# ming024/FastSpeech2

Hardware: AMD Instinct MI355X
Metric: mel-frames/sec (train, 80-bin) (higher is better)
Workload: dtype bf16; 1 GPU; BASELINE configs[1]: LJSpeech train, 4+4 FFT layers d=256 2 heads, 80-bin mel, batch=48/GPU, L=128 phonemes, T=925 frames, fwd+loss+bwd+clip+Adam, dropout on, fp32 master weights; global_batch=48, parallelism=dp1, hip_graph=False, side_stream_wgrad=True, windows=1, library=fastspeech2_amd/libfs2hip.so

## Files before the change

fastspeech2_amd/csrc/fs2_common.h:

```cpp
#pragma once
#include <hip/hip_runtime.h>
#include <stdint.h>
#include <stdio.h>
#include <mutex>
#include <stdlib.h>

#define FS2_OK 0
#define FS2_EINVAL (-1)
#define FS2_EDTYPE (-2)
#define FS2_ELAUNCH (-3)

enum { FS2_F32 = 0, FS2_BF16 = 1 };
enum { FS2_ACT_NONE = 0, FS2_ACT_RELU = 1, FS2_ACT_TANH = 2, FS2_ACT_LRELU = 3, FS2_ACT_GATE = 4 };

void fs2_set_error(const char* fmt, ...);

#define FS2_CHECK_ARG(cond, ...)                \
    do {                                        \
        if (!(cond)) {                          \
            fs2_set_error(__VA_ARGS__);         \
            return FS2_EINVAL;                  \
        }                                       \
    } while (0)

struct Fs2DevOnce {
    std::mutex mu;
    uint64_t done = 0;
    template <typename F>
    void run(F&& f) {
        int d = 0;
        (void)hipGetDevice(&d);
        const uint64_t bit = 1ull << (d & 63);
        std::lock_guard<std::mutex> g(mu);
        if (!(done & bit)) { f(); done |= bit; }
    }
};

#define FS2_CHECK_LAUNCH(name)                                                        \
    do {                                                                              \
        hipError_t e__ = hipGetLastError();                                           \
        if (e__ != hipSuccess) {                                                      \
            fs2_set_error("%s: launch failed: %s", name, hipGetErrorString(e__));     \
            return FS2_ELAUNCH;                                                       \
        }                                                                             \
    } while (0)

typedef uint16_t bf16_t;

__device__ __forceinline__ float bf16_to_f32(bf16_t v) { return __uint_as_float(((uint32_t)v) << 16); }
typedef __bf16 fs2_bf16x2 __attribute__((ext_vector_type(2)));
typedef float fs2_f32x2 __attribute__((ext_vector_type(2)));
__device__ __forceinline__ bf16_t f32_to_bf16(float f) { return __builtin_bit_cast(unsigned short, (__bf16)f); }
__device__ __forceinline__ uint32_t pack_bf16x2(float lo, float hi) {
    return __builtin_bit_cast(uint32_t, __builtin_convertvector((fs2_f32x2){lo, hi}, fs2_bf16x2));
}

template <typename T> struct Elem;
template <> struct Elem<float> {
    static __device__ __forceinline__ float ld(const float* p) { return *p; }
    static __device__ __forceinline__ void st(float* p, float v) { *p = v; }
};
template <> struct Elem<bf16_t> {
    static __device__ __forceinline__ float ld(const bf16_t* p) { return bf16_to_f32(*p); }
    static __device__ __forceinline__ void st(bf16_t* p, float v) { *p = f32_to_bf16(v); }
};

template <typename T> __device__ __forceinline__ float4 ld4(const T* p);
template <> __device__ __forceinline__ float4 ld4<float>(const float* p) { return *reinterpret_cast<const float4*>(p); }
template <> __device__ __forceinline__ float4 ld4<bf16_t>(const bf16_t* p) {
    uint2 u = *reinterpret_cast<const uint2*>(p);
    float4 r;
    r.x = __uint_as_float(u.x << 16);
    r.y = __uint_as_float(u.x & 0xffff0000u);
    r.z = __uint_as_float(u.y << 16);
    r.w = __uint_as_float(u.y & 0xffff0000u);
    return r;
}
template <typename T> __device__ __forceinline__ void st4(T* p, float4 v);
template <> __device__ __forceinline__ void st4<float>(float* p, float4 v) { *reinterpret_cast<float4*>(p) = v; }
template <> __device__ __forceinline__ void st4<bf16_t>(bf16_t* p, float4 v) {
    uint2 u;
    u.x = pack_bf16x2(v.x, v.y);
    u.y = pack_bf16x2(v.z, v.w);
    *reinterpret_cast<uint2*>(p) = u;
}

__device__ __forceinline__ float wave_sum(float v) {
#pragma unroll
    for (int o = 32; o > 0; o >>= 1) v += __shfl_xor(v, o, 64);
    return v;
}
__device__ __forceinline__ float wave_max(float v) {
#pragma unroll
    for (int o = 32; o > 0; o >>= 1) v = fmaxf(v, __shfl_xor(v, o, 64));
    return v;
}

__device__ __forceinline__ uint32_t fs2_hash32(uint32_t x) {
    x ^= x >> 16; x *= 0x7feb352du;
    x ^= x >> 15; x *= 0x846ca68bu;
    x ^= x >> 16;
    return x;
}
__device__ __forceinline__ float fs2_uniform(uint64_t seed, uint32_t idx) {
    uint32_t h = fs2_hash32(idx ^ (uint32_t)seed);
    h = fs2_hash32(h + (uint32_t)(seed >> 32) + 0x9e3779b9u);
    return (float)(h >> 8) * (1.0f / 16777216.0f);
}
__device__ __forceinline__ float fs2_drop_scale(uint64_t seed, uint32_t idx, float p, float inv_keep) {
    return (fs2_uniform(seed, idx) >= p) ? inv_keep : 0.0f;
}

#ifndef FS2_GEMM_PLAIN
#define FS2_GEMM_PLAIN 1
#define FS2_GEMM_DMA 2
#define FS2_GEMM_RING 3
#define FS2_GEMM_SKINNY 4
#define FS2_GEMM_PERSIST 5
#define FS2_GEMM_PERSIST_1TAP 6
#define FS2_GEMM_WIDE_1TAP 7
#define FS2_GEMM_STREAM_K256 9
#endif
static inline int fs2_cdiv(long a, long b) { return (int)((a + b - 1) / b); }
```

fastspeech2_amd/csrc/fs2_gemm.hip:

```cpp
#include "fs2_common.h"
#include <stdlib.h>
#include <type_traits>

#include "fs2_gemm.h"
#include "fs2_sched.h"
#include "fs2_wgrad.h"

template <typename T> __host__ __device__ __forceinline__ int fs2_tile_col128(int c) { return fs2_tile_col128_bytes((int)sizeof(T), c); }
template <typename T, int TW = 128, int NT = 256, int ROWS = 128>
__device__ __forceinline__ void gemm_store_tile(const ConvGemmArgs& a, const float* tile, int m0, int n0, int tid) {
    constexpr int EPC = MmaTraits<T>::EPC;
    T* Y = reinterpret_cast<T*>(a.Y);
    const T* R = reinterpret_cast<const T*>(a.R);
    constexpr int EPT = EPC;
    constexpr int CPR = TW / EPT;
    const bool gate = a.act == FS2_ACT_GATE;
#pragma unroll 4
    for (int it = 0; it < (ROWS * CPR) / NT; ++it) {
        int idx = tid + NT * it;
        int rl = idx / CPR, cc = (idx % CPR) * EPT;
        int m = m0 + rl, n = n0 + cc;
        if (m >= a.M || n >= a.N) continue;
        float v[EPT];
#pragma unroll
// ... 497 lines not shown

template <bool ONE_TAP, bool MASK, bool INACT>
__device__ __forceinline__ void ring_consumer(const ConvGemmArgs& a, unsigned char* smem, f32x16 (&acc)[2][2], int m0, int lane,
                                              int wm, int wn) {
    typedef RingCfg<ONE_TAP> C;
    constexpr int D = C::D;
    const int nkc = a.Cin >> 6;
    const int taps = ONE_TAP ? 1 : a.taps;
    const int nsteps = taps * nkc;
    const int fl = lane & 31, fh = lane >> 5;
    unsigned boff[4];
#pragma unroll
    for (int j = 0; j < 4; ++j) {
        int r = wn * 64 + fl;
        boff[j] = r * 128 + (((fh * 4 + j) ^ ((r >> 1) & 7)) << 4);
    }
    unsigned vmask[2] = {0, 0};
    if (MASK) {
#pragma unroll
        for (int mb = 0; mb < 2; ++mb) {
            int m = m0 + wm * 64 + mb * 32 + fl;
            unsigned msk = 0;
            if (m < a.M) {
                int t = m % a.S;
                for (int j = 0; j < taps; ++j) {
                    int ts = t + j * a.dil - a.pad;
                    if (ts >= 0 && ts < a.S) msk |= 1u << j;
                }
            }
            vmask[mb] = msk;
        }
    }
    typedef unsigned u32x4 __attribute__((ext_vector_type(4)));
#define FS2_DS_READ_B128(dst, addr, OFF) asm volatile("ds_read_b128 %0, %1 offset:" #OFF : "=v"(dst) : "v"(addr))
    u32x4 af[2][2][2], bf[2][2][2];
    const unsigned smem_u = lds_addr(smem);
    auto read_group = [&](int set, int kc, int tap, int slot, int g) {
        const int roff = tap * a.dil;
        const unsigned a_base = (ONE_TAP ? slot : (kc & 1)) * C::A_BYTES + (wm * 64 + roff) * 128;
        const unsigned x = ((fl + roff) >> 1) & 7;
#pragma unroll
        for (int q = 0; q < 2; ++q) {
            const int j = 2 * g + q;
            const unsigned aaddr = smem_u + a_base + fl * 128 + ((((unsigned)(fh * 4 + j)) ^ x) << 4);
            const unsigned baddr = smem_u + C::B_OFF + slot * RING_B_BYTES + boff[j];
            FS2_DS_READ_B128(bf[set][q][0], baddr, 0);
            FS2_DS_READ_B128(bf[set][q][1], baddr, 4096);
            FS2_DS_READ_B128(af[set][q][0], aaddr, 0);
            FS2_DS_READ_B128(af[set][q][1], aaddr, 4096);
        }
    };
    auto mfma_group = [&](int set, int tap) {
#pragma unroll
        for (int q = 0; q < 2; ++q)
#pragma unroll
            for (int mb = 0; mb < 2; ++mb) {
                u32x4 av = af[set][q][mb];
                if (INACT) {
#pragma unroll
                    for (int e = 0; e < 4; ++e) {
                        float lo = __uint_as_float(av[e] << 16), hi = __uint_as_float(av[e] & 0xffff0000u);
                        av[e] = pack_bf16x2(fmaxf(lo, lo * a.in_slope), fmaxf(hi, hi * a.in_slope));
                    }
                }
                if (MASK && !((vmask[mb] >> tap) & 1u)) av = u32x4{0u, 0u, 0u, 0u};
#pragma unroll
                for (int nb = 0; nb < 2; ++nb)
                    acc[mb][nb] = __builtin_amdgcn_mfma_f32_32x32x16_bf16(
                        __builtin_bit_cast(bf16x8, av), __builtin_bit_cast(bf16x8, bf[set][q][nb]), acc[mb][nb], 0, 0, 0);
            }
    };
    asm volatile("s_waitcnt lgkmcnt(0)" ::: "memory");
    __builtin_amdgcn_s_barrier();
    read_group(0, 0, 0, 0, 0);
    int slot = 0, step = 0;
    for (int kc = 0; kc < nkc; ++kc) {
        for (int tap = 0; tap < taps; ++tap, ++step) {
            read_group(1, kc, tap, slot, 1);
            asm volatile("s_waitcnt lgkmcnt(8)" ::: "memory");
            __builtin_amdgcn_sched_barrier(0);
            mfma_group(0, tap);
            __builtin_amdgcn_sched_barrier(0);
            int nslot = slot + 1; if (nslot == D) nslot = 0;
            int ntap = tap + 1, nkc_ = kc; if (ntap == taps) { ntap = 0; ++nkc_; }
            asm volatile("s_waitcnt lgkmcnt(0)" ::: "memory");
            if (step + 1 < nsteps) {
                __builtin_amdgcn_s_barrier();
                read_group(0, nkc_, ntap, nslot, 0);
            }
            __builtin_amdgcn_sched_barrier(0);
            mfma_group(1, tap);
            __builtin_amdgcn_sched_barrier(0);
            slot = nslot;
        }
    }
#undef FS2_DS_READ_B128
}

template <bool ONE_TAP, bool INACT>
__global__ void __launch_bounds__(768, 3) conv_gemm_ring_kernel(ConvGemmArgs a) {
    extern __shared__ __attribute__((aligned(16))) unsigned char smem[];
    const int tid = threadIdx.x, lane = tid & 63;
    const int wave = __builtin_amdgcn_readfirstlane(tid >> 6);
    const int wm = (wave >> 1) & 3, wn = wave & 1;
    const int ntm = (a.M + 255) >> 8;
    const int tile_m = blockIdx.x % ntm, tile_n = blockIdx.x / ntm;
    const int m0 = tile_m * 256, n0 = tile_n * 128;
    bf16_t* Y = reinterpret_cast<bf16_t*>(a.Y);

    if (a.lens) {
        int mlast = min(m0 + 255, a.M - 1);
        int b0 = m0 / a.S, b1 = mlast / a.S;
        if (b0 == b1 && (m0 - b0 * a.S) >= a.lens[b0]) {
            if (!a.accumulate) {
                for (int i = tid; i < 256 * 16; i += 768) {
                    int r = i >> 4, c = (i & 15) * 8;
                    int m = m0 + r, n = n0 + c;
                    if (m >= a.M || n >= a.N) continue;
                    bf16_t* yp = Y + (size_t)m * a.ldy + n;
                    if (a.vec_ok && n + 8 <= a.N) *reinterpret_cast<uint4*>(yp) = make_uint4(0, 0, 0, 0);
                    else for (int e = 0; e < 8 && n + e < a.N; ++e) yp[e] = 0;
                }
            }
            return;
        }
    }
    f32x16 acc[2][2];
    if (wave >= 8) {
        ring_loader<ONE_TAP>(a, smem, m0, n0, lane, wave - 8);
    } else {
#pragma unroll
        for (int i = 0; i < 2; ++i)
#pragma unroll
            for (int j = 0; j < 2; ++j)
#pragma unroll
                for (int r = 0; r < 16; ++r) acc[i][j][r] = 0.f;
        if (ONE_TAP) {
            ring_consumer<true, false, INACT>(a, smem, acc, m0, lane, wm, wn);
        } else {
            int t0 = m0 % a.S;
            int rows = min(256, a.M - m0);
            const bool need_mask = (t0 < a.pad) || (t0 + rows - 1 + (a.taps - 1) * a.dil - a.pad >= a.S);
            if (need_mask) ring_consumer<false, true, INACT>(a, smem, acc, m0, lane, wm, wn);
            else ring_consumer<false, false, INACT>(a, smem, acc, m0, lane, wm, wn);
        }
    }
    __syncthreads();

    float* tile = reinterpret_cast<float*>(smem);
    if (wave < 8) {
        const int fl = lane & 31, fh = lane >> 5;
        auto stage = [&](auto actc) {
            constexpr int ACT = decltype(actc)::value;
#pragma unroll
            for (int nb = 0; nb < 2; ++nb) {
                int cl = wn * 64 + nb * 32 + fl;
                int n = n0 + cl;
                float bv = (a.bias && n < a.N) ? a.bias[n] : 0.f;
#pragma unroll
                for (int mb = 0; mb < 2; ++mb)
#pragma unroll
                    for (int r = 0; r < 16; ++r) {
                        int rl = wm * 64 + mb * 32 + (r & 3) + 8 * (r >> 2) + 4 * fh;
                        tile[rl * 128 + fs2_tile_col128<bf16_t>(cl)] = act_ct<ACT>(acc[mb][nb][r] + bv, a.slope);
                    }
            }
        };
        FS2_ACT_DISPATCH(a.act, stage(std::integral_constant<int, ACT>{}));
    }
    __syncthreads();
    if (tid < 512) {
        gemm_store_tile<bf16_t, 128, 512>(a, tile, m0, n0, tid);
        gemm_store_tile<bf16_t, 128, 512>(a, tile + 128 * 128, m0 + 128, n0, tid);
    }
}

template <int C> struct SkinnyCfg {
    static constexpr int CPR = C / 8, RPW = 16 / CPR, XR_MAX = 192;
    static constexpr int G = C == 32 ? 8 : 2;
    static constexpr int X_BYTES = XR_MAX * C * 2, W_BYTES = G * C * C * 2;
    static constexpr int EPI_BYTES = 128 * C * 4;
    static constexpr int LDS = (X_BYTES + W_BYTES) > EPI_BYTES ? (X_BYTES + W_BYTES) : EPI_BYTES;
};
template <int C> __device__ __forceinline__ unsigned skinny_swz(int row, int c) {
    typedef SkinnyCfg<C> K;
    return (unsigned)(row * (C * 2) + ((c ^ ((row / K::RPW) % K::CPR)) << 4));
}

template <int C>
__global__ void __launch_bounds__(256) conv_skinny_kernel(ConvGemmArgs a) {
    typedef SkinnyCfg<C> K;
    constexpr int CPR = K::CPR, NB = C / 32, NS = C / 16;
    extern __shared__ __attribute__((aligned(16))) unsigned char smem[];
    unsigned char* sX = smem;
    unsigned char* sW = smem + K::X_BYTES;
    const int tid = threadIdx.x, lane = tid & 63, fl = lane & 31, fh = lane >> 5;
    const int wave = __builtin_amdgcn_readfirstlane(tid >> 6);
    const int m0 = blockIdx.x * 128;
    const bf16_t* X = reinterpret_cast<const bf16_t*>(a.X);
    const bf16_t* W = reinterpret_cast<const bf16_t*>(a.W);
    const int halo = (a.taps - 1) * a.dil;
    const int xr = 128 + halo;
    constexpr int MAXI = (K::XR_MAX * CPR + 255) / 256;
    uint4 xv[MAXI];
#pragma unroll
    for (int i = 0; i < MAXI; ++i) {
        const int idx = tid + 256 * i;
        const int row = idx / CPR, c = idx % CPR;
        const int g = m0 - a.pad + row;
        uint4 v = make_uint4(0, 0, 0, 0);
        if (row < xr && g >= 0 && g < a.M) v = *reinterpret_cast<const uint4*>(X + (size_t)g * a.ldx + c * 8);
        xv[i] = v;
    }
#pragma unroll
    for (int i = 0; i < MAXI; ++i) {
        const int idx = tid + 256 * i;
        const int row = idx / CPR, c = idx % CPR;
        if (row < xr) {
            uint4 v = xv[i];
            if (a.in_act == FS2_ACT_LRELU) v = act_chunk_bf16(v, a.in_slope);
            *reinterpret_cast<uint4*>(sX + skinny_swz<C>(row, c)) = v;
        }
    }
    unsigned vmask = 0;
    {
        const int m = m0 + wave * 32 + fl;
        if (m < a.M) {
            const int t = m % a.S;
            for (int j = 0; j < a.taps; ++j) {
                const int ts = t + j * a.dil - a.pad;
                if (ts >= 0 && ts < a.S) vmask |= 1u << j;
            }
        }
    }
    f32x16 acc[NB];
#pragma unroll
    for (int nb = 0; nb < NB; ++nb)
#pragma unroll
        for (int r = 0; r < 16; ++r) acc[nb][r] = 0.f;

    constexpr int WI = (K::G * C * CPR) / 256;
    for (int g0 = 0; g0 < a.taps; g0 += K::G) {
        __syncthreads();
#pragma unroll
        for (int i = 0; i < WI; ++i) {
            const int idx = tid + 256 * i;
            const int tl = idx / (C * CPR), rem = idx % (C * CPR);
            const int n = rem / CPR, c = rem % CPR;
            uint4 v = make_uint4(0, 0, 0, 0);
            if (g0 + tl < a.taps) v = *reinterpret_cast<const uint4*>(W + ((size_t)n * a.taps + (g0 + tl)) * C + c * 8);
            *reinterpret_cast<uint4*>(sW + tl * (C * C * 2) + skinny_swz<C>(n, c)) = v;
        }
        __syncthreads();
#pragma unroll
        for (int tl = 0; tl < K::G; ++tl) {
            const int tap = g0 + tl;
            if (tap >= a.taps) break;
            const int r = wave * 32 + fl + tap * a.dil;
            const bool live = (vmask >> tap) & 1u;
            const unsigned char* wt = sW + tl * (C * C * 2);
#pragma unroll
            for (int sl = 0; sl < NS; ++sl) {
                const int c = 2 * sl + fh;
                uint4 av = *reinterpret_cast<const uint4*>(sX + skinny_swz<C>(r, c));
                if (!live) av = make_uint4(0, 0, 0, 0);
#pragma unroll
                for (int nb = 0; nb < NB; ++nb) {
                    uint4 bv = *reinterpret_cast<const uint4*>(wt + skinny_swz<C>(nb * 32 + fl, c));
                    acc[nb] = __builtin_amdgcn_mfma_f32_32x32x16_bf16(__builtin_bit_cast(bf16x8, av), __builtin_bit_cast(bf16x8, bv), acc[nb], 0, 0, 0);
                }
            }
        }
    }
    __syncthreads();
    float* tile = reinterpret_cast<float*>(smem);
    auto stage = [&](auto actc) {
        constexpr int ACT = decltype(actc)::value;
#pragma unroll
        for (int nb = 0; nb < NB; ++nb) {
            const int cl = nb * 32 + fl;
            const float bv = a.bias ? a.bias[cl] : 0.f;
#pragma unroll
            for (int r = 0; r < 16; ++r) {
                const int rl = wave * 32 + (r & 3) + 8 * (r >> 2) + 4 * fh;
                tile[rl * C + cl] = act_ct<ACT>(acc[nb][r] + bv, a.slope);
            }
        }
    };
    FS2_ACT_DISPATCH(a.act, stage(std::integral_constant<int, ACT>{}));
    __syncthreads();
    gemm_store_tile<bf16_t, C, 256, 128>(a, tile, m0, 0, tid);
}

template <int C>
static void launch_skinny(const ConvGemmArgs& a, hipStream_t stream) {
    static Fs2DevOnce once;
    once.run([&] { (void)hipFuncSetAttribute((const void*)conv_skinny_kernel<C>, hipFuncAttributeMaxDynamicSharedMemorySize, SkinnyCfg<C>::LDS); });
    conv_skinny_kernel<C><<<(unsigned)fs2_cdiv(a.M, 128), 256, SkinnyCfg<C>::LDS, stream>>>(a);
}

bool fs2_conv_gemm_w_ok(const ConvGemmArgs& a, bool has_map, int dtype);
void fs2_conv_gemm_w_launch(const ConvGemmArgs& a, const int32_t* tile_map, hipStream_t stream);
bool fs2_conv_gemm_p_ok(const ConvGemmArgs& a, bool has_map, int dtype, int ks);
void fs2_conv_gemm_p_launch(const ConvGemmArgs& a, const int32_t* tile_map, hipStream_t stream, int ks, float* ws, float* tail_ws);

bool fs2_conv_gemm_s_ok(const ConvGemmArgs& a, int dtype);
void fs2_conv_gemm_s_launch(const ConvGemmArgs& a, hipStream_t stream);
struct GemmPick { int variant; bool ring_inact, ks2; };
static GemmPick conv_gemm_pick(const ConvGemmArgs& a, int dtype, bool has_map, bool has_tail_ws = true) {
    const int M = a.M, N = a.N, Cin = a.Cin, taps = a.taps, dil = a.dil, in_act = a.in_act;
    GemmPick p;
    const long grid = (long)fs2_cdiv(M, 128) * fs2_cdiv(N, 128);
    const bool dma = in_act == FS2_ACT_NONE && (taps > 1 || (grid <= 160 && Cin % 128 == 0 && Cin >= 768 && dtype == FS2_BF16)) && (taps - 1) * dil <= 16 && taps <= 32;
    const long big_tiles = (long)fs2_cdiv(M, 256) * fs2_cdiv(N, 128);
    p.ring_inact = in_act == FS2_ACT_LRELU && a.in_slope > 0.f && a.in_slope < 1.f;
    const bool ring_ok = dtype == FS2_BF16 && (in_act == FS2_ACT_NONE || p.ring_inact) && (taps == 1 || (taps >= 3 && (taps - 1) * dil <= 16 && taps <= 32)) &&
                         Cin % 64 == 0 && (double)M * a.ldx * 2 < 2.0e9 && (double)N * taps * Cin * 2 < 2.0e9;
    const bool big = ring_ok && big_tiles >= 170 && (taps > 1 || Cin >= 1024);
    const bool skinny = dtype == FS2_BF16 && N == Cin && (Cin == 32 || Cin == 64) && taps <= 16 &&
                        (taps - 1) * dil <= 64 && (in_act == FS2_ACT_NONE || in_act == FS2_ACT_LRELU) && a.vec_ok;
    const bool res_short = (a.res_unlrelu > 0.f || a.post_slope > 0.f) && (a.R || a.accumulate) && a.act != FS2_ACT_GATE &&
                           (long)taps * ((Cin + 63) / 64) <= 48 && big;
    const bool persist = !skinny && !res_short && fs2_conv_gemm_p_ok(a, has_map, dtype, 1) && (taps > 1 || Cin >= 256);
    p.ks2 = dtype == FS2_BF16 && grid <= 160 && Cin % 128 == 0 && (long)taps * (Cin / 64) >= 12;
    const bool lrelu_io = a.res_unlrelu > 0.f || a.post_slope > 0.f;
    if (!skinny && !lrelu_io && fs2_conv_gemm_s_ok(a, dtype)) { p.variant = FS2_GEMM_STREAM_K256; return p; }
    if (!skinny && fs2_conv_gemm_w_ok(a, has_map, dtype)) { p.variant = FS2_GEMM_WIDE_1TAP; return p; }
    p.variant = skinny ? FS2_GEMM_SKINNY : (persist ? (taps == 1 ? FS2_GEMM_PERSIST_1TAP : FS2_GEMM_PERSIST) : (big ? FS2_GEMM_RING : (dma ? FS2_GEMM_DMA : FS2_GEMM_PLAIN)));
    return p;
}

static void conv_gemm_fill(ConvGemmArgs& a, const void* X, long ldx, const void* W, const float* bias, const void* R, long ldr, void* Y,
                           long ldy, const int32_t* lens, int M, int N, int Cin, int S, int taps, int dil, int pad, int act, float slope,
                           int in_act, float in_slope, int accumulate, float out_scale, int dtype) {
    const int epc = dtype == FS2_F32 ? 4 : 8;
    a.X = X; a.ldx = ldx; a.W = W; a.ldw = (long)taps * Cin; a.bias = bias; a.R = R; a.ldr = ldr; a.Y = Y; a.ldy = ldy;
    a.lens = lens; a.M = M; a.N = N; a.Cin = Cin; a.S = S; a.taps = taps; a.dil = dil; a.pad = pad; a.act = act;
    a.slope = slope; a.in_act = in_act; a.in_slope = in_slope; a.accumulate = accumulate; a.out_scale = out_scale;
    a.res_unlrelu = 0.f; a.post_slope = 0.f;
    a.vec_ok = (ldy % epc == 0) && (((uintptr_t)Y & 15) == 0) && (!R || ((ldr % epc == 0) && (((uintptr_t)R & 15) == 0)));
}

extern "C" int fs2_conv_gemm_variant(long ldx, long ldy, long ldr, int has_lens, int has_map, int M, int N, int Cin, int S, int taps,
                                     int dil, int in_act, float in_slope, int dtype) {
    ConvGemmArgs a;
    conv_gemm_fill(a, nullptr, ldx, nullptr, nullptr, ldr ? (const void*)16 : nullptr, ldr, nullptr, ldy, has_lens ? (const int32_t*)16 : nullptr,
                   M, N, Cin, S > 0 ? S : 1, taps, dil, 0, 0, 0.f, in_act, in_slope, 0, 1.f, dtype);
    return conv_gemm_pick(a, dtype, has_map != 0).variant;
}

extern "C" int fs2_conv_gemm_lrelu_io_variant(long ldx, long ldy, long ldr, int accumulate, int M, int N, int Cin, int S, int taps, int dil,
                                              int act, float res_unlrelu, float post_slope, int dtype) {
    ConvGemmArgs a;
    conv_gemm_fill(a, nullptr, ldx, nullptr, nullptr, ldr ? (const void*)16 : nullptr, ldr, nullptr, ldy, nullptr, M, N, Cin, S > 0 ? S : 1,
                   taps, dil, 0, act, 0.f, FS2_ACT_NONE, 0.f, accumulate, 1.f, dtype);
    a.res_unlrelu = res_unlrelu; a.post_slope = post_slope;
    return conv_gemm_pick(a, dtype, false).variant;
}

static int conv_gemm_impl(const void* X, long ldx, const void* W, const float* bias, const void* R, long ldr, void* Y,
                          long ldy, const int32_t* lens, const int32_t* tile_map, float* tail_ws, int M, int N, int Cin, int S, int taps,
                          int dil, int pad, int act, float slope, int in_act, float in_slope, int accumulate, float out_scale,
                          int dtype, hipStream_t stream, float res_unlrelu = 0.f, float post_slope = 0.f) {
    FS2_CHECK_ARG(X && W && Y, "conv_gemm: null pointer");
    FS2_CHECK_ARG(M >= 0 && N > 0 && Cin > 0 && S > 0 && taps > 0 && dil > 0, "conv_gemm: bad shape M=%d N=%d Cin=%d S=%d taps=%d", M, N, Cin, S, taps);
    FS2_CHECK_ARG(M % S == 0, "conv_gemm: M=%d not a multiple of S=%d", M, S);
    int epc = dtype == FS2_F32 ? 4 : 8;
    FS2_CHECK_ARG(dtype == FS2_F32 || dtype == FS2_BF16, "conv_gemm: dtype %d", dtype);
    FS2_CHECK_ARG(Cin % epc == 0 && ldx % epc == 0, "conv_gemm: Cin=%d / ldx=%ld must be multiples of %d", Cin, ldx, epc);
    FS2_CHECK_ARG(((uintptr_t)X & 15) == 0 && ((uintptr_t)W & 15) == 0, "conv_gemm: X/W must be 16-byte aligned");
    if (M == 0) return FS2_OK;
    ConvGemmArgs a;
    conv_gemm_fill(a, X, ldx, W, bias, R, ldr, Y, ldy, lens, M, N, Cin, S, taps, dil, pad, act, slope, in_act, in_slope, accumulate, out_scale, dtype);
    FS2_CHECK_ARG(res_unlrelu >= 0.f && post_slope >= 0.f && post_slope < 1.f && (res_unlrelu == 0.f || (R && act != FS2_ACT_GATE)),
                  "conv_gemm: res_unlrelu needs an additive residual operand, post_slope in [0, 1)");
    a.res_unlrelu = res_unlrelu; a.post_slope = post_slope;
    const long grid = (long)fs2_cdiv(M, 128) * fs2_cdiv(N, 128);
    const long big_tiles = (long)fs2_cdiv(M, 256) * fs2_cdiv(N, 128);
    const GemmPick pk = conv_gemm_pick(a, dtype, tile_map != nullptr, tail_ws != nullptr);
    if (pk.variant == FS2_GEMM_STREAM_K256) {
        fs2_conv_gemm_s_launch(a, stream);
    } else if (pk.variant == FS2_GEMM_SKINNY) {
        if (Cin == 32) launch_skinny<32>(a, stream);
        else launch_skinny<64>(a, stream);
    } else if (pk.variant == FS2_GEMM_WIDE_1TAP) {
        fs2_conv_gemm_w_launch(a, tile_map, stream);
    } else if (pk.variant == FS2_GEMM_PERSIST || pk.variant == FS2_GEMM_PERSIST_1TAP) {
        fs2_conv_gemm_p_launch(a, tile_map, stream, 1, nullptr, tail_ws);
    } else if (pk.variant == FS2_GEMM_RING) {
        static Fs2DevOnce ring_once;
        const int dyn1 = RingCfg<true>::B_OFF + RingCfg<true>::D * RING_B_BYTES;
        const int dynk = RingCfg<false>::B_OFF + RingCfg<false>::D * RING_B_BYTES;
        ring_once.run([&] {
            (void)hipFuncSetAttribute((const void*)conv_gemm_ring_kernel<true, false>, hipFuncAttributeMaxDynamicSharedMemorySize, dyn1);
            (void)hipFuncSetAttribute((const void*)conv_gemm_ring_kernel<false, false>, hipFuncAttributeMaxDynamicSharedMemorySize, dynk);
            (void)hipFuncSetAttribute((const void*)conv_gemm_ring_kernel<true, true>, hipFuncAttributeMaxDynamicSharedMemorySize, dyn1);
            (void)hipFuncSetAttribute((const void*)conv_gemm_ring_kernel<false, true>, hipFuncAttributeMaxDynamicSharedMemorySize, dynk);
        });
        if (pk.ring_inact) {
            if (taps == 1) conv_gemm_ring_kernel<true, true><<<(unsigned)big_tiles, 768, dyn1, stream>>>(a);
            else conv_gemm_ring_kernel<false, true><<<(unsigned)big_tiles, 768, dynk, stream>>>(a);
        } else if (taps == 1) conv_gemm_ring_kernel<true, false><<<(unsigned)big_tiles, 768, dyn1, stream>>>(a);
        else conv_gemm_ring_kernel<false, false><<<(unsigned)big_tiles, 768, dynk, stream>>>(a);
    } else if (pk.variant == FS2_GEMM_DMA) {
        const int dyn = 2 * 160 * 128 + 2 * 128 * 128;
        static Fs2DevOnce dma_once;
        dma_once.run([&] {
            (void)hipFuncSetAttribute((const void*)conv_gemm_dma_kernel<float, 1>, hipFuncAttributeMaxDynamicSharedMemorySize, dyn);
            (void)hipFuncSetAttribute((const void*)conv_gemm_dma_kernel<bf16_t, 1>, hipFuncAttributeMaxDynamicSharedMemorySize, dyn);
            (void)hipFuncSetAttribute((const void*)conv_gemm_dma_kernel<bf16_t, 2>, hipFuncAttributeMaxDynamicSharedMemorySize, 2 * dyn);
        });
        if (dtype == FS2_F32) conv_gemm_dma_kernel<float, 1><<<(unsigned)grid, 256, dyn, stream>>>(a);
        else if (pk.ks2) conv_gemm_dma_kernel<bf16_t, 2><<<(unsigned)grid, 512, 2 * dyn, stream>>>(a);
        else conv_gemm_dma_kernel<bf16_t, 1><<<(unsigned)grid, 256, dyn, stream>>>(a);
    } else if (dtype == FS2_F32) conv_gemm_kernel<float><<<(unsigned)grid, 256, 0, stream>>>(a);
    else conv_gemm_kernel<bf16_t><<<(unsigned)grid, 256, 0, stream>>>(a);
    FS2_CHECK_LAUNCH("conv_gemm");
    return FS2_OK;
}

extern "C" int fs2_conv_gemm(const void* X, long ldx, const void* W, const float* bias, const void* R, long ldr, void* Y,
                             long ldy, const int32_t* lens, const int32_t* tile_map, int M, int N, int Cin, int S, int taps, int dil,
                             int pad, int act, float slope, int in_act, float in_slope, int accumulate, float out_scale, int dtype,
                             hipStream_t stream) {
    return conv_gemm_impl(X, ldx, W, bias, R, ldr, Y, ldy, lens, tile_map, nullptr, M, N, Cin, S, taps, dil, pad, act, slope, in_act,
                          in_slope, accumulate, out_scale, dtype, stream);
}

extern "C" int fs2_conv_gemm_tail(const void* X, long ldx, const void* W, const float* bias, const void* R, long ldr, void* Y,
                                  long ldy, const int32_t* lens, const int32_t* tile_map, float* tail_ws, int M, int N, int Cin,
                                  int S, int taps, int dil, int pad, int act, float slope, int in_act, float in_slope,
                                  int accumulate, float out_scale, int dtype, hipStream_t stream) {
    FS2_CHECK_ARG(!tail_ws || ((uintptr_t)tail_ws & 15) == 0, "conv_gemm_tail: tail_ws must be 16-byte aligned");
    return conv_gemm_impl(X, ldx, W, bias, R, ldr, Y, ldy, lens, tile_map, tail_ws, M, N, Cin, S, taps, dil, pad, act, slope, in_act,
                          in_slope, accumulate, out_scale, dtype, stream);
}

extern "C" int fs2_conv_gemm_lrelu_io(const void* X, long ldx, const void* W, const float* bias, const void* R, long ldr, void* Y,
                                      long ldy, float* tail_ws, int M, int N, int Cin, int S, int taps, int dil, int pad, int act,
                                      float slope, int accumulate, float out_scale, float res_unlrelu, float post_slope, int dtype,
                                      hipStream_t stream) {
    FS2_CHECK_ARG(!tail_ws || ((uintptr_t)tail_ws & 15) == 0, "conv_gemm_lrelu_io: tail_ws must be 16-byte aligned");
    return conv_gemm_impl(X, ldx, W, bias, R, ldr, Y, ldy, nullptr, nullptr, tail_ws, M, N, Cin, S, taps, dil, pad, act, slope,
                          FS2_ACT_NONE, 0.f, accumulate, out_scale, dtype, stream, res_unlrelu, post_slope);
}

extern "C" int fs2_conv_gemm_splitk(const void* X, long ldx, const void* W, const float* bias, const void* R, long ldr, void* Y,
                                    long ldy, const int32_t* lens, const int32_t* tile_map, float* ws, int ksplit, int M, int N,
                                    int Cin, int S, int taps, int dil, int pad, int act, float slope, float out_scale, int dtype,
                                    hipStream_t stream) {
    FS2_CHECK_ARG(X && W && Y && ws, "conv_gemm_splitk: null pointer");
    FS2_CHECK_ARG(M > 0 && N > 0 && Cin > 0 && S > 0 && taps > 0 && dil > 0 && M % S == 0 && ksplit >= 2, "conv_gemm_splitk: bad shape");
    FS2_CHECK_ARG(((uintptr_t)X & 15) == 0 && ((uintptr_t)W & 15) == 0 && ((uintptr_t)ws & 15) == 0 && ldx % 8 == 0, "conv_gemm_splitk: alignment");
    ConvGemmArgs a;
    conv_gemm_fill(a, X, ldx, W, bias, R, ldr, Y, ldy, lens, M, N, Cin, S, taps, dil, pad, act, slope, FS2_ACT_NONE, 0.f, 0, out_scale, dtype);
    FS2_CHECK_ARG(fs2_conv_gemm_p_ok(a, tile_map != nullptr, dtype, ksplit), "conv_gemm_splitk: shape not supported (M=%d N=%d Cin=%d taps=%d ksplit=%d)", M, N, Cin, taps, ksplit);
    fs2_conv_gemm_p_launch(a, tile_map, stream, ksplit, ws, nullptr);
    FS2_CHECK_LAUNCH("conv_gemm_splitk");
    return FS2_OK;
}

template <typename T>
__global__ void pack_weight_kernel(const float* __restrict__ w, T* __restrict__ wf, T* __restrict__ wd, int Cout, int Cin, int k) {
    size_t total = (size_t)Cout * Cin * k;
    for (size_t i = (size_t)blockIdx.x * blockDim.x + threadIdx.x; i < total; i += (size_t)gridDim.x * blockDim.x) {
        int c = (int)(i % Cin);
        size_t q = i / Cin;
        int j = (int)(q % k);
        int n = (int)(q / k);
        float v = w[i];
        if (wf) Elem<T>::st(wf + i, v);
        if (wd) Elem<T>::st(wd + ((size_t)c * k + (k - 1 - j)) * Cout + n, v);
    }
}
extern "C" int fs2_pack_weight(const float* w, void* wf, void* wd, int Cout, int Cin, int k, int dtype, hipStream_t stream) {
    FS2_CHECK_ARG(w && (wf || wd), "pack_weight: null pointer");
    size_t total = (size_t)Cout * Cin * k;
    if (total == 0) return FS2_OK;
    int grid = (int)((total + 255) / 256 < 4096 ? (total + 255) / 256 : 4096);
    if (dtype == FS2_F32) pack_weight_kernel<float><<<grid, 256, 0, stream>>>(w, (float*)wf, (float*)wd, Cout, Cin, k);
    else if (dtype == FS2_BF16) pack_weight_kernel<bf16_t><<<grid, 256, 0, stream>>>(w, (bf16_t*)wf, (bf16_t*)wd, Cout, Cin, k);
    else { fs2_set_error("pack_weight: dtype"); return FS2_EDTYPE; }
    FS2_CHECK_LAUNCH("pack_weight");
    return FS2_OK;
}

template <typename T>
__global__ void __launch_bounds__(256) pack_dgrad_multi_kernel(const float* __restrict__ flat, T* __restrict__ wd_base,
                                                               const int64_t* __restrict__ table, int n_entries) {
    __shared__ float tile[64][65];
    int e = 0;
    while (e + 1 < n_entries && (int)table[(e + 1) * 6 + 5] <= (int)blockIdx.x) ++e;
    const int64_t* d = table + e * 6;
    const float* w = flat + d[0];
    T* wd = wd_base + d[1];
    const int Cout = (int)d[2], Cin = (int)d[3], k = (int)d[4];
    int t = (int)blockIdx.x - (int)d[5];
    const int tn = (Cout + 63) >> 6, tc = (Cin + 63) >> 6;
    const int in_ = t % tn; t /= tn;
    const int ic = t % tc; t /= tc;
    const int j = t;
    const int n0 = in_ * 64, c0 = ic * 64;
    const int lx = threadIdx.x & 63, ly = threadIdx.x >> 6;
#pragma unroll 4
    for (int r = ly; r < 64; r += 4) {
        int n = n0 + r, c = c0 + lx;
        tile[r][lx] = (n < Cout && c < Cin) ? w[((size_t)n * k + j) * Cin + c] : 0.f;
    }
    __syncthreads();
#pragma unroll 4
    for (int r = ly; r < 64; r += 4) {
        int c = c0 + r, n = n0 + lx;
        if (c < Cin && n < Cout) Elem<T>::st(wd + ((size_t)c * k + (k - 1 - j)) * Cout + n, tile[lx][r]);
    }
}
extern "C" int fs2_pack_dgrad_multi(const float* flat, void* wd_base, const int64_t* table, int n_entries, int total_tiles,
                                    int dtype, hipStream_t stream) {
    FS2_CHECK_ARG(flat && wd_base && table, "pack_dgrad_multi: null pointer");
    if (n_entries <= 0 || total_tiles <= 0) return FS2_OK;
    if (dtype == FS2_F32) pack_dgrad_multi_kernel<float><<<total_tiles, 256, 0, stream>>>(flat, (float*)wd_base, table, n_entries);
    else if (dtype == FS2_BF16) pack_dgrad_multi_kernel<bf16_t><<<total_tiles, 256, 0, stream>>>(flat, (bf16_t*)wd_base, table, n_entries);
    else { fs2_set_error("pack_dgrad_multi: dtype"); return FS2_EDTYPE; }
    FS2_CHECK_LAUNCH("pack_dgrad_multi");
    return FS2_OK;
}


template <typename T>
__global__ void __launch_bounds__(256, 2) conv_wgrad_kernel(WgradArgs a) {
    __shared__ __attribute__((aligned(16))) float sA[2][32][128];
    __shared__ __attribute__((aligned(16))) float sB[2][32][128];
    const int tid = threadIdx.x, lane = tid & 63, wave = tid >> 6;
    const int wm = wave >> 1, wn = wave & 1;
    const int ntn = (a.N + 127) >> 7, ntc = (a.Cin + 127) >> 7;
    int bx = blockIdx.x;
    const int tile_n = bx % ntn; bx /= ntn;
    const int tile_c = bx % ntc; bx /= ntc;
    const int tap = bx;
    const int n0 = tile_n * 128, c0 = tile_c * 128;
    const int shift = tap * a.dil - a.pad;
    const int mbeg = blockIdx.y * a.rows_per_split;
    const int mend = min(a.M, mbeg + a.rows_per_split);
    if (mbeg >= mend) return;
    const T* dY = reinterpret_cast<const T*>(a.dY);
    const T* X = reinterpret_cast<const T*>(a.X);

    const int sr = tid >> 5, sc4 = (tid & 31) * 4;
    float4 ra[4], rb[4];
    auto load_tile = [&](int mt) {
#pragma unroll
        for (int i = 0; i < 4; ++i) {
            int m = mt + sr + 8 * i;
            float4 va = make_float4(0.f, 0.f, 0.f, 0.f), vb = va;
            if (m < mend) {
                int n = n0 + sc4;
                if (n < a.N) va = ld4<T>(dY + (size_t)m * a.lddy + n);
                int t = m % a.S, ts = t + shift;
                int c = c0 + sc4;
                if (ts >= 0 && ts < a.S && c < a.Cin) vb = ld4<T>(X + (size_t)(m + shift) * a.ldx + c);
            }
            ra[i] = va; rb[i] = vb;
        }
    };
    auto store_tile = [&](int buf) {
#pragma unroll
        for (int i = 0; i < 4; ++i) {
            *reinterpret_cast<float4*>(&sA[buf][sr + 8 * i][sc4]) = ra[i];
            *reinterpret_cast<float4*>(&sB[buf][sr + 8 * i][sc4]) = rb[i];
        }
    };
    f32x16 acc[2][2];
#pragma unroll
    for (int i = 0; i < 2; ++i)
#pragma unroll
        for (int j = 0; j < 2; ++j)
#pragma unroll
            for (int r = 0; r < 16; ++r) acc[i][j][r] = 0.f;
    const int fl = lane & 31, fh = lane >> 5;
    int nt = (mend - mbeg + 31) / 32;
    load_tile(mbeg);
    store_tile(0);
    __syncthreads();
    for (int it = 0; it < nt; ++it) {
        if (it + 1 < nt) load_tile(mbeg + (it + 1) * 32);
        int buf = it & 1;
#pragma unroll
        for (int ks = 0; ks < 16; ++ks) {
            float af[2], bf[2];
            int row = ks * 2 + fh;
#pragma unroll
            for (int mb = 0; mb < 2; ++mb) af[mb] = sA[buf][row][wm * 64 + mb * 32 + fl];
#pragma unroll
            for (int nb = 0; nb < 2; ++nb) bf[nb] = sB[buf][row][wn * 64 + nb * 32 + fl];
#pragma unroll
            for (int mb = 0; mb < 2; ++mb)
#pragma unroll
                for (int nb = 0; nb < 2; ++nb)
                    acc[mb][nb] = __builtin_amdgcn_mfma_f32_32x32x2f32(af[mb], bf[nb], acc[mb][nb], 0, 0, 0);
        }
        if (it + 1 < nt) store_tile((it + 1) & 1);
        __syncthreads();
    }
#pragma unroll
    for (int nb = 0; nb < 2; ++nb) {
        int c = c0 + wn * 64 + nb * 32 + fl;
        if (c >= a.Cin) continue;
#pragma unroll
        for (int mb = 0; mb < 2; ++mb)
#pragma unroll
            for (int r = 0; r < 16; ++r) {
                int n = n0 + wm * 64 + mb * 32 + (r & 3) + 8 * (r >> 2) + 4 * fh;
                if (n >= a.N) continue;
                atomicAdd(a.dW + ((size_t)n * a.taps + tap) * a.Cin + c, acc[mb][nb][r]);
            }
    }
}


typedef short s16x4 __attribute__((ext_vector_type(4)));
typedef short s16x8 __attribute__((ext_vector_type(8)));

__device__ __forceinline__ uint4 and4(uint4 v, unsigned m) { return make_uint4(v.x & m, v.y & m, v.z & m, v.w & m); }
__device__ __forceinline__ int wg_swz(int row, int c16) { return row * 256 + ((((c16 >> 2) ^ (row & 3))) << 6) + ((c16 & 3) << 4); }

template <int NT, int NW>
__device__ __forceinline__ void wgrad_bf16_body(const WgradArgs& a, unsigned char* smem, int tile_n, int tile_c, int tap0) {
    constexpr int XROWS = 64 + 8;
    constexpr int A_BYTES = 64 * 256, X_BYTES = XROWS * 256;
    const int tid = threadIdx.x, lane = tid & 63;
    const int wave = __builtin_amdgcn_readfirstlane(tid >> 6);
    constexpr int NBC = NW == 4 ? 2 : 1;
    constexpr int RS = NW * 4, NI = 64 / RS;
    const int wm = NW == 4 ? (wave >> 1) : (wave >> 2), wn = NW == 4 ? (wave & 1) : (wave & 3);
    const int n0 = tile_n * 128, c0 = tile_c * 128;
    const int shift0 = tap0 * a.dil - a.pad;
    const int tps = (a.S + 63) >> 6;
    const int nunits = (a.M / a.S) * tps;
    const int ubeg = blockIdx.y * a.rows_per_split;
    const int uend = min(nunits, ubeg + a.rows_per_split);
    if (ubeg >= uend) return;
    const bf16_t* dY = reinterpret_cast<const bf16_t*>(a.dY);
    const bf16_t* X = reinterpret_cast<const bf16_t*>(a.X);

    const int sr = tid >> 4, sc = tid & 15;
    const bool ncol_ok = (n0 + sc * 8) < a.N, ccol_ok = (c0 + sc * 8) < a.Cin;
    const int ncol = ncol_ok ? n0 + sc * 8 : 0, ccol = ccol_ok ? c0 + sc * 8 : 0;
    const bool x5 = wave < 2;
    uint4 ra[2][NI], rb[2][NI], rb4[2] = {make_uint4(0, 0, 0, 0), make_uint4(0, 0, 0, 0)};
    bool live_t[2] = {false, false};
    const bool do_bias = a.dbias != nullptr && tile_c == 0 && tap0 == 0;
    float bsum[8] = {0.f, 0.f, 0.f, 0.f, 0.f, 0.f, 0.f, 0.f};
    const bool col_full = (n0 + 128 <= a.N) && (c0 + 128 <= a.Cin);
    const unsigned char* dYb = reinterpret_cast<const unsigned char*>(dY);
    const unsigned char* Xb = reinterpret_cast<const unsigned char*>(X);
    const unsigned dy_rs = (unsigned)a.lddy * 2u, x_rs = (unsigned)a.ldx * 2u;
    unsigned okmask_t[2] = {0, 0};
    bool edge_t[2] = {false, false};
    auto load_tile = [&](auto setc, int u) {
        constexpr int SET = decltype(setc)::value;
        const bool valid = u < uend;
        const int uu = valid ? u : ubeg;
        const int seq = uu / tps, t0 = (uu - seq * tps) * 64;
        const int tend = a.lens ? min(a.lens[seq], a.S) : a.S;
        live_t[SET] = valid && t0 < tend;
        edge_t[SET] = !col_full || (t0 + 64 > tend) || (t0 + shift0 < 0) || (t0 + shift0 + XROWS > a.S);
        const unsigned base = (unsigned)(seq * a.S);
        unsigned ok = 0;
#pragma unroll
        for (int i = 0; i < NI; ++i) {
            const int t = t0 + sr + RS * i;
            const size_t o = (size_t)(base + (unsigned)min(t, a.S - 1)) * dy_rs + (unsigned)ncol * 2u;
            ra[SET][i] = *reinterpret_cast<const uint4*>(dYb + o);
            ok |= (ncol_ok && t < tend) ? (1u << i) : 0u;
        }
#pragma unroll
        for (int i = 0; i < NI; ++i) {
            const int t = t0 + shift0 + sr + RS * i;
            const size_t o = (size_t)(base + (unsigned)min(max(t, 0), a.S - 1)) * x_rs + (unsigned)ccol * 2u;
            rb[SET][i] = *reinterpret_cast<const uint4*>(Xb + o);
            ok |= (ccol_ok && t >= 0 && t < a.S) ? (16u << i) : 0u;
        }
        {
            const int t = t0 + shift0 + sr + 64;
            const size_t o = (size_t)(base + (unsigned)min(max(t, 0), a.S - 1)) * x_rs + (unsigned)ccol * 2u;
            rb4[SET] = *reinterpret_cast<const uint4*>(Xb + o);
            ok |= (ccol_ok && t >= 0 && t < a.S) ? 256u : 0u;
        }
        okmask_t[SET] = ok;
    };
    auto store_tile = [&](auto setc, int buf) {
        constexpr int SET = decltype(setc)::value;
        const unsigned okmask = okmask_t[SET];
        unsigned char* As = smem + buf * (A_BYTES + X_BYTES);
        unsigned char* Bs = As + A_BYTES;
        if (edge_t[SET]) {
#pragma unroll
            for (int i = 0; i < NI; ++i) ra[SET][i] = and4(ra[SET][i], 0u - ((okmask >> i) & 1u));
#pragma unroll
            for (int i = 0; i < NI; ++i) rb[SET][i] = and4(rb[SET][i], 0u - ((okmask >> (4 + i)) & 1u));
            rb4[SET] = and4(rb4[SET], 0u - ((okmask >> 8) & 1u));
        }
#pragma unroll
        for (int i = 0; i < NI; ++i) *reinterpret_cast<uint4*>(As + wg_swz(sr + RS * i, sc)) = ra[SET][i];
#pragma unroll
        for (int i = 0; i < NI; ++i) *reinterpret_cast<uint4*>(Bs + wg_swz(sr + RS * i, sc)) = rb[SET][i];
        if (x5) *reinterpret_cast<uint4*>(Bs + wg_swz(sr + 64, sc)) = rb4[SET];
        if (do_bias) {
#pragma unroll
            for (int i = 0; i < NI; ++i) {
                const uint32_t* u32 = reinterpret_cast<const uint32_t*>(&ra[SET][i]);
#pragma unroll
                for (int e = 0; e < 4; ++e) {
                    bsum[2 * e] += __uint_as_float(u32[e] << 16);
                    bsum[2 * e + 1] += __uint_as_float(u32[e] & 0xffff0000u);
                }
            }
        }
    };
    f32x16 acc[NT][2][NBC];
#pragma unroll
    for (int t = 0; t < NT; ++t)
#pragma unroll
        for (int i = 0; i < 2; ++i)
#pragma unroll
            for (int j = 0; j < NBC; ++j)
#pragma unroll
                for (int r = 0; r < 16; ++r) acc[t][i][j][r] = 0.f;
    const int li = lane & 15, g = lane >> 4, h = g >> 1;
    const int rrow = 8 * h + (li >> 2);
    const int acol = wm * 64 + 16 * (g & 1) + 4 * (li & 3);
    const int bcol = wn * (32 * NBC) + 16 * (g & 1) + 4 * (li & 3);
    typedef __attribute__((address_space(3))) s16x4* lds_s4;
    auto tr_off = [&](int row, int col) -> unsigned { return (unsigned)(row * 256 + ((((col >> 5) ^ (row & 3))) << 6) + ((col & 31) << 1)); };
    unsigned offA[2][2], offB[NT][NBC][2];
#pragma unroll
    for (int blk = 0; blk < 2; ++blk)
#pragma unroll
        for (int hl = 0; hl < 2; ++hl) {
            offA[blk][hl] = tr_off(rrow + 4 * hl, acol + blk * 32);
            if (blk < NBC) {
#pragma unroll
                for (int t = 0; t < NT; ++t) offB[t][blk][hl] = A_BYTES + tr_off(rrow + 4 * hl + t * a.dil, bcol + blk * 32);
            }
        }
    const unsigned smem_u = (unsigned)(size_t)(__attribute__((address_space(3))) unsigned char*)smem;
    auto tr_read = [&](unsigned off) -> s16x4 {
        return __builtin_amdgcn_ds_read_tr16_b64_v4i16((lds_s4)(size_t)(smem_u + off));
    };
    s16x8 af[2][2], bf[2][NT][NBC];
    auto read_frags = [&](int set, int bufoff, int ks) {
#pragma unroll
        for (int blk = 0; blk < 2; ++blk) {
            s16x4 lo = tr_read(offA[blk][0] + bufoff + ks * 4096);
            s16x4 hi = tr_read(offA[blk][1] + bufoff + ks * 4096);
            af[set][blk] = __builtin_shufflevector(lo, hi, 0, 1, 2, 3, 4, 5, 6, 7);
        }
#pragma unroll
        for (int t = 0; t < NT; ++t)
#pragma unroll
            for (int blk = 0; blk < NBC; ++blk) {
                s16x4 lo = tr_read(offB[t][blk][0] + bufoff + ks * 4096);
// ... 268 lines not shown
```

fastspeech2_amd/csrc/fs2_gemm_p.hip:

```cpp
#include "fs2_gemm.h"
#include "fs2_sched.h"
#include "fs2_gemm_epi.h"


template <bool ONE_TAP, bool WIDE> struct PCfg;
template <> struct PCfg<false, false> {
    static constexpr int D = 5, HALO = 16, A_BYTES = 272 * 128, SCRATCH = 2 * 272 * 128, B_OFF = 2 * 272 * 128 + 1024, NJA = 9;
    static constexpr int AUX = B_OFF + D * 16384;
};
template <> struct PCfg<false, true> {
    static constexpr int D = 4, HALO = 64, A_BYTES = 320 * 128, SCRATCH = 2 * 320 * 128, B_OFF = 2 * 320 * 128 + 1024, NJA = 10;
    static constexpr int AUX = B_OFF + D * 16384;
};
template <> struct PCfg<true, false> {
    static constexpr int D = 3, HALO = 0, A_BYTES = 256 * 128, SCRATCH = 0, B_OFF = 3 * 256 * 128, NJA = 8;
    static constexpr int AUX = B_OFF + D * 16384;
};
__device__ __forceinline__ const unsigned char* p_uniform(const unsigned char* q) {
    const unsigned long long u = reinterpret_cast<unsigned long long>(q);
    const unsigned lo = __builtin_amdgcn_readfirstlane((unsigned)u), hi = __builtin_amdgcn_readfirstlane((unsigned)(u >> 32));
    return reinterpret_cast<const unsigned char*>(((unsigned long long)hi << 32) | lo);
}
template <int N> __device__ __forceinline__ void p_wait_vm() { asm volatile("s_waitcnt vmcnt(%0)" :: "n"(N) : "memory"); }
static constexpr int P_MAXB = 1024;
static constexpr int P_AUX_BYTES = P_MAXB * 4 + 8 * 512;
static constexpr int P_B_BYTES = 128 * 128;

__device__ __forceinline__ int p_ntiles(const PSched& s) {
    const PPlan p = p_plan(s, s.b);
    return p.R + (p.j < p.tail * p.tks ? 1 : 0);
}
__device__ __forceinline__ int p_last_nkc(const PSched& s) {
    const PPlan p = p_plan(s, s.b);
    return (p.j < p.tail * p.tks) ? s.nkc_u / p.tks : s.nkc_u;
}

struct PUnits { unsigned v0, v1; };
__device__ __forceinline__ void p_units_load(const PSched& s, int lane, PUnits& t) {
    int mi, nt, kc0, nkc, np;
    unsigned a0 = 0, a1 = 0;
    if (p_unit(s, lane, mi, nt, kc0, nkc, np)) {
        const int mt = s.tmap ? s.tmap[1 + mi] : mi;
        a0 = (unsigned)mt | ((unsigned)nt << 20) | ((unsigned)np << 28);
        a1 = (unsigned)kc0 | ((unsigned)nkc << 16);
    }
    t.v0 = a0; t.v1 = a1;
}
__device__ __forceinline__ void p_tile_of(const PSched& s, int k, const PUnits& t, int& mt, int& nt, int& kc0, int* split = nullptr,
                                          int* nparts = nullptr) {
    const unsigned a0 = __builtin_amdgcn_readlane(t.v0, k), a1 = __builtin_amdgcn_readlane(t.v1, k);
    mt = (int)(a0 & 0xfffffu);
    nt = (int)((a0 >> 20) & 0xffu);
    kc0 = __builtin_amdgcn_readfirstlane((int)(a1 & 0xffffu));
    if (nparts) *nparts = (int)(a0 >> 28);
    if (split) *split = kc0 / s.nkc_u;
}

template <bool ONE_TAP, bool WIDE>
__device__ __forceinline__ void p_loader(const ConvGemmArgs& a, const PSched& sc, unsigned char* smem, int lane, int lw,
                                         const PUnits& units, int ntiles) {
    typedef PCfg<ONE_TAP, WIDE> C;
    constexpr int D = C::D, NJA = C::NJA;
    const unsigned char* Xb = reinterpret_cast<const unsigned char*>(a.X);
    const unsigned char* Wb = reinterpret_cast<const unsigned char*>(a.W);
    const int nkc = sc.nkc_u;
    const int nkc_last = p_last_nkc(sc);
    const int taps = ONE_TAP ? 1 : a.taps;
    const int nsteps = taps * nkc;
    const int total = (ntiles - 1) * nsteps + taps * nkc_last;
    const int nchunks = (ntiles - 1) * nkc + nkc_last;
    int kc0A = 0, kc0B = 0;
    const int lr = lane >> 3, lc = lane & 7;
    const int arows = 256 + (taps - 1) * a.dil;
    const unsigned smem_base = lds_addr(smem);

    unsigned offA[NJA], ldsA[NJA], offB[4];
    auto set_A = [&](int k) {
        int mt, nt;
        p_tile_of(sc, k, units, mt, nt, kc0A);
        const int m0 = mt * 256;
#pragma unroll
        for (int j = 0; j < NJA; ++j) {
            const int wl = lw + 4 * j;
            const bool live = wl * 8 < arows;
            const int r = wl * 8 + lr;
            const int g = min(max(m0 - a.pad + r, 0), a.M - 1);
            offA[j] = live ? (unsigned)g * (unsigned)(a.ldx * 2) + (unsigned)((lc ^ ((r >> 1) & 7)) << 4) : 0u;
            ldsA[j] = live ? (unsigned)(wl * 1024) : 0xffffffffu;
        }
    };
    auto set_B = [&](int k) {
        int mt, nt;
        p_tile_of(sc, k, units, mt, nt, kc0B);
        const int n0 = nt * 128;
#pragma unroll
        for (int j = 0; j < 4; ++j) {
            const int r = (lw * 4 + j) * 8 + lr;
            const int n = min(n0 + r, a.N - 1);
            offB[j] = (unsigned)n * (unsigned)(a.ldw * 2) + (unsigned)((lc ^ ((r >> 1) & 7)) << 4);
        }
    };
    int is = 0, ik = 0, ikc = 0, itap = 0, islot = 0;
    int kA = -1, kB = -1;
    auto issue_A = [&](int k, int kc, int buf_or_slot) {
        if (k != kA) { set_A(k); kA = k; }
        const unsigned char* base = p_uniform(Xb + (size_t)(kc0A + kc) * 128);
#pragma unroll
        for (int j = 0; j < NJA; ++j) {
            const unsigned d = (ldsA[j] == 0xffffffffu) ? smem_base + C::SCRATCH : smem_base + buf_or_slot * C::A_BYTES + ldsA[j];
            glds16_sbase(offA[j], base, __builtin_amdgcn_readfirstlane(d));
        }
    };
    auto issue_step = [&]() {
        if (ik != kB) { set_B(ik); kB = ik; }
        if (ONE_TAP) issue_A(ik, ikc, islot);
        const unsigned char* base = p_uniform(Wb + ((size_t)itap * a.Cin + (size_t)(kc0B + ikc) * 64) * 2);
        const unsigned d0 = smem_base + C::B_OFF + islot * P_B_BYTES + lw * 4096;
#pragma unroll
        for (int j = 0; j < 4; ++j) glds16_sbase(offB[j], base, d0 + j * 1024);
    };
    auto advance_issue = [&]() {
        ++is;
        if (++itap == taps) { itap = 0; if (++ikc == (ik == ntiles - 1 ? nkc_last : nkc)) { ikc = 0; ++ik; } }
        if (++islot == D) islot = 0;
    };
    if (!ONE_TAP) issue_A(0, 0, 0);
#pragma unroll
    for (int p = 0; p < D - 1; ++p) {
        if (is < total) issue_step();
        advance_issue();
    }
    int ck = 0, ckc = 0, ctap = 0, gc = 0;
    for (int cs = 0; cs < total; ++cs) {
        if (total - 1 - cs < D - 2) {
            asm volatile("s_waitcnt vmcnt(0)" ::: "memory");
        } else if (ONE_TAP) {
            p_wait_vm<(D - 2) * (NJA + 4)>();
        } else {
            const bool a_young = (ctap >= 1 && ctap <= D - 2) && (gc + 1 < nchunks);
            if (a_young) p_wait_vm<(D - 2) * 4 + NJA>();
            else p_wait_vm<(D - 2) * 4>();
        }
        __builtin_amdgcn_s_barrier();
        if (!ONE_TAP && ctap == 0 && gc + 1 < nchunks) {
            int nk = ck, nkc_ = ckc + 1;
            if (nkc_ == (ck == ntiles - 1 ? nkc_last : nkc)) { nkc_ = 0; ++nk; }
            issue_A(nk, nkc_, (gc + 1) & 1);
        }
        if (is < total) issue_step();
        advance_issue();
        if (++ctap == taps) { ctap = 0; ++gc; if (++ckc == (ck == ntiles - 1 ? nkc_last : nkc)) { ckc = 0; ++ck; } }
    }
}

#define FS2P_DS_READ(dst, addr, OFF) asm volatile("ds_read_b128 %0, %1 offset:" #OFF : "=v"(dst) : "v"(addr))
#define FS2P_WAIT_LGKM(N) asm volatile("s_waitcnt lgkmcnt(" #N ")" ::: "memory")
#define FS2P_FENCE() __builtin_amdgcn_sched_barrier(0)

template <int MB>
__device__ __forceinline__ void p_epilogue_splitk(const ConvGemmArgs& a, float* ws, f32x16 (&acc)[MB][4], int m0, int n0, int wm,
                                                  int fl, int fh) {
#pragma unroll
    for (int mb = 0; mb < MB; ++mb) {
        const int m = m0 + wm * (32 * MB) + mb * 32 + fl;
        if (m >= a.M) continue;
        float* wrow = ws + (size_t)m * a.N;
#pragma unroll
        for (int nb = 0; nb < 4; ++nb) {
            float c[2][8];
#pragma unroll
            for (int e = 0; e < 4; ++e) {
                u32x2 s0 = __builtin_amdgcn_permlane32_swap(__float_as_uint(acc[mb][nb][e]), __float_as_uint(acc[mb][nb][4 + e]), false, false);
                u32x2 s1 = __builtin_amdgcn_permlane32_swap(__float_as_uint(acc[mb][nb][8 + e]), __float_as_uint(acc[mb][nb][12 + e]), false, false);
                c[0][e] = __uint_as_float(s0[0]); c[0][4 + e] = __uint_as_float(s0[1]);
                c[1][e] = __uint_as_float(s1[0]); c[1][4 + e] = __uint_as_float(s1[1]);
            }
#pragma unroll
            for (int ch = 0; ch < 2; ++ch) {
                const int n = n0 + nb * 32 + ch * 16 + fh * 8;
                if (n >= a.N) continue;
                *reinterpret_cast<float4*>(wrow + n) = make_float4(c[ch][0], c[ch][1], c[ch][2], c[ch][3]);
                *reinterpret_cast<float4*>(wrow + n + 4) = make_float4(c[ch][4], c[ch][5], c[ch][6], c[ch][7]);
            }
        }
    }
}

template <int ACT>
__global__ void __launch_bounds__(256) splitk_finalize_kernel(ConvGemmArgs a, const float* __restrict__ ws, int ks) {
    const int cpr = a.N >> 3;
    const long idx = (long)blockIdx.x * 256 + threadIdx.x;
    if (idx >= (long)a.M * cpr) return;
    const int m = (int)(idx / cpr), n = (int)(idx - (long)m * cpr) * 8;
    const float* wp = ws + (size_t)m * a.N + n;
    const size_t slab = (size_t)a.M * a.N;
    float v[8] = {0.f, 0.f, 0.f, 0.f, 0.f, 0.f, 0.f, 0.f};
    for (int sp = 0; sp < ks; ++sp) {
        const float4 x0 = *reinterpret_cast<const float4*>(wp + sp * slab), x1 = *reinterpret_cast<const float4*>(wp + sp * slab + 4);
        v[0] += x0.x; v[1] += x0.y; v[2] += x0.z; v[3] += x0.w; v[4] += x1.x; v[5] += x1.y; v[6] += x1.z; v[7] += x1.w;
    }
    if (a.bias) {
#pragma unroll
        for (int e = 0; e < 8; ++e) v[e] += a.bias[n + e];
    }
#pragma unroll
    for (int e = 0; e < 8; ++e) v[e] = act_ct<ACT>(v[e], a.slope);
    const bool gate = a.act == FS2_ACT_GATE;
    if (a.R) {
        const uint4 rv = *reinterpret_cast<const uint4*>(reinterpret_cast<const bf16_t*>(a.R) + (size_t)m * a.ldr + n);
        const uint32_t* u = reinterpret_cast<const uint32_t*>(&rv);
#pragma unroll
        for (int e = 0; e < 4; ++e) {
            float r0 = __uint_as_float(u[e] << 16), r1 = __uint_as_float(u[e] & 0xffff0000u);
            if (a.res_unlrelu > 0.f) { r0 = r0 > 0.f ? r0 : r0 * a.res_unlrelu; r1 = r1 > 0.f ? r1 : r1 * a.res_unlrelu; }
            v[2 * e] = gate ? (r0 > 0.f ? v[2 * e] : 0.f) : v[2 * e] + r0;
            v[2 * e + 1] = gate ? (r1 > 0.f ? v[2 * e + 1] : 0.f) : v[2 * e + 1] + r1;
        }
    }
    bool padrow = false;
    if (a.lens) { const int b = m / a.S; padrow = (m - b * a.S) >= a.lens[b]; }
    uint4 o;
    uint32_t* ou = reinterpret_cast<uint32_t*>(&o);
#pragma unroll
    for (int e = 0; e < 4; ++e) {
        float x0 = v[2 * e] * a.out_scale, x1 = v[2 * e + 1] * a.out_scale;
        if (a.post_slope > 0.f) { x0 = x0 > 0.f ? x0 : x0 * a.post_slope; x1 = x1 > 0.f ? x1 : x1 * a.post_slope; }
        ou[e] = padrow ? 0u : pack_bf16x2(x0, x1);
    }
    *reinterpret_cast<uint4*>(reinterpret_cast<bf16_t*>(a.Y) + (size_t)m * a.ldy + n) = o;
}

template <int MB>
__device__ __forceinline__ void p_epilogue_part(float* slab, f32x16 (&acc)[MB][4], int wm, int fl, int fh) {
#pragma unroll
    for (int mb = 0; mb < MB; ++mb) {
        float* wrow = slab + (size_t)(wm * (32 * MB) + mb * 32 + fl) * 128;
#pragma unroll
        for (int nb = 0; nb < 4; ++nb) {
            float c[2][8];
#pragma unroll
            for (int e = 0; e < 4; ++e) {
                u32x2 s0 = __builtin_amdgcn_permlane32_swap(__float_as_uint(acc[mb][nb][e]), __float_as_uint(acc[mb][nb][4 + e]), false, false);
                u32x2 s1 = __builtin_amdgcn_permlane32_swap(__float_as_uint(acc[mb][nb][8 + e]), __float_as_uint(acc[mb][nb][12 + e]), false, false);
                c[0][e] = __uint_as_float(s0[0]); c[0][4 + e] = __uint_as_float(s0[1]);
                c[1][e] = __uint_as_float(s1[0]); c[1][4 + e] = __uint_as_float(s1[1]);
            }
#pragma unroll
            for (int ch = 0; ch < 2; ++ch) {
                const int n = nb * 32 + ch * 16 + fh * 8;
                *reinterpret_cast<float4*>(wrow + n) = make_float4(c[ch][0], c[ch][1], c[ch][2], c[ch][3]);
                *reinterpret_cast<float4*>(wrow + n + 4) = make_float4(c[ch][4], c[ch][5], c[ch][6], c[ch][7]);
            }
        }
    }
}

template <int ACT>
__global__ void __launch_bounds__(256) p_tail_finalize_kernel(ConvGemmArgs a, PSched sc) {
    const int i = blockIdx.y;
    sc.b = sc.order == 0 ? 2 * i : (i & 7) + 8 * (2 * (i >> 3));
    if (sc.b >= sc.G) return;
    if (sc.tmap) { sc.n_real = sc.tmap[0]; sc.n_pad = sc.ntm - sc.n_real; }
    const PPlan p = p_plan(sc, sc.b);
    if (p.tks <= 1 || p.j >= p.tail * p.tks || (p.j % p.tks) != 0) return;
    int mi, nt, sp;
    p_pos(sc, p, p.R * p.Gg + p.j / p.tks, mi, nt, sp);
    const int mt = sc.tmap ? sc.tmap[1 + mi] : mi;
    const bool gate = a.act == FS2_ACT_GATE;
#pragma unroll
  for (int pass = 0; pass < 4; ++pass) {
    const int idx = (blockIdx.x * 4 + pass) * 256 + threadIdx.x;
    const int r = idx >> 4, cn = (idx & 15) * 8;
    const int m = mt * 256 + r, n = nt * 128 + cn;
    if (m >= a.M || n >= a.N) continue;
    float v[8] = {0.f, 0.f, 0.f, 0.f, 0.f, 0.f, 0.f, 0.f};
    for (int q = 0; q < p.tks; ++q) {
        const int wg = sc.order == 0 ? sc.b + q : p.x + 8 * (p.j + q);
        const float* sl = sc.tws + (size_t)wg * (256 * 128) + r * 128 + cn;
        const float4 x0 = *reinterpret_cast<const float4*>(sl), x1 = *reinterpret_cast<const float4*>(sl + 4);
        v[0] += x0.x; v[1] += x0.y; v[2] += x0.z; v[3] += x0.w; v[4] += x1.x; v[5] += x1.y; v[6] += x1.z; v[7] += x1.w;
    }
    if (a.bias) {
#pragma unroll
        for (int e = 0; e < 8; ++e) v[e] += a.bias[n + e];
    }
#pragma unroll
    for (int e = 0; e < 8; ++e) v[e] = act_ct<ACT>(v[e], a.slope);
    if (a.R) {
        const uint4 rv = *reinterpret_cast<const uint4*>(reinterpret_cast<const bf16_t*>(a.R) + (size_t)m * a.ldr + n);
        const uint32_t* u = reinterpret_cast<const uint32_t*>(&rv);
#pragma unroll
        for (int e = 0; e < 4; ++e) {
            float r0 = __uint_as_float(u[e] << 16), r1 = __uint_as_float(u[e] & 0xffff0000u);
            if (a.res_unlrelu > 0.f) { r0 = r0 > 0.f ? r0 : r0 * a.res_unlrelu; r1 = r1 > 0.f ? r1 : r1 * a.res_unlrelu; }
            v[2 * e] = gate ? (r0 > 0.f ? v[2 * e] : 0.f) : v[2 * e] + r0;
            v[2 * e + 1] = gate ? (r1 > 0.f ? v[2 * e + 1] : 0.f) : v[2 * e + 1] + r1;
        }
    }
    bool padrow = false;
    if (a.lens) { const int b = m / a.S; padrow = (m - b * a.S) >= a.lens[b]; }
    uint4 o;
    uint32_t* ou = reinterpret_cast<uint32_t*>(&o);
#pragma unroll
    for (int e = 0; e < 4; ++e) {
        float x0 = v[2 * e] * a.out_scale, x1 = v[2 * e + 1] * a.out_scale;
        if (a.post_slope > 0.f) { x0 = x0 > 0.f ? x0 : x0 * a.post_slope; x1 = x1 > 0.f ? x1 : x1 * a.post_slope; }
        ou[e] = padrow ? 0u : pack_bf16x2(x0, x1);
    }
    *reinterpret_cast<uint4*>(reinterpret_cast<bf16_t*>(a.Y) + (size_t)m * a.ldy + n) = o;
  }
}

__device__ __forceinline__ u32x4 p_lrelu(u32x4 v, float slope) {
#pragma unroll
    for (int e = 0; e < 4; ++e) {
        const float lo = __uint_as_float(v[e] << 16), hi = __uint_as_float(v[e] & 0xffff0000u);
        v[e] = pack_bf16x2(fmaxf(lo, lo * slope), fmaxf(hi, hi * slope));
    }
    return v;
}

template <bool ONE_TAP, bool WIDE, int INACT, int MB>
__device__ __forceinline__ void p_consumer(const ConvGemmArgs& a, const PSched& sc, unsigned char* smem, int lane, int wm,
                                           const PUnits& units, int ntiles, const int32_t* lens_s, float* bias_s) {
    typedef PCfg<ONE_TAP, WIDE> C;
    constexpr int D = C::D;
    const int nkc = sc.nkc_u;
    const int nkc_last = p_last_nkc(sc);
    const int taps = ONE_TAP ? 1 : a.taps;
    const int nsteps = taps * nkc;
    const int total = (ntiles - 1) * nsteps + taps * nkc_last;
    const int fl = lane & 31, fh = lane >> 5;
    const unsigned smem_u = lds_addr(smem);
    const unsigned c0 = (unsigned)(fh * 4);
    const unsigned ckb = c0 ^ (unsigned)((fl >> 1) & 7);
    const unsigned blane = smem_u + C::B_OFF + (unsigned)(fl * 128);
    const unsigned alane = smem_u + (unsigned)((wm * (32 * MB) + fl) * 128);
    auto a_base = [&](int abuf, int tap) -> unsigned { return alane + (unsigned)(abuf * C::A_BYTES + tap * a.dil * 128); };
    auto a_key = [&](int tap) -> unsigned { return c0 ^ (unsigned)(((fl + tap * a.dil) >> 1) & 7); };
    auto b_base = [&](int slot) -> unsigned { return blane + (unsigned)(slot * P_B_BYTES); };

    u32x4 Af[2][MB], Bf[2][4];
    f32x16 acc[MB][4];

#define FS2P_MFMA(SET, MB, NB, AV)                                                                                      \
    acc[MB][NB] = __builtin_amdgcn_mfma_f32_32x32x16_bf16(__builtin_bit_cast(bf16x8, Bf[SET][NB]), __builtin_bit_cast(bf16x8, AV), \
                                                          acc[MB][NB], 0, 0, 0)
#define FS2P_SLICE(SET, MASKED, LIVE0, LIVE1, JN, ABASE, AKEY, BBASE)                                                   \
    do {                                                                                                                \
        u32x4 av0, av1;                                                                                                 \
        FS2P_WAIT_LGKM(4); FS2P_FENCE();                                                                                \
        av0 = Af[SET][0]; if (INACT) av0 = p_lrelu(av0, a.in_slope);                                                    \
        if (MASKED && !(LIVE0)) av0 = u32x4{0u, 0u, 0u, 0u};                                                            \
        FS2P_MFMA(SET, 0, 0, av0); FS2P_FENCE();                                                                        \
        const unsigned aa_ = (ABASE) + ((((AKEY)) ^ (unsigned)(JN)) << 4);                                              \
        const unsigned ba_ = (BBASE) + ((ckb ^ (unsigned)(JN)) << 4);                                                   \
        FS2P_DS_READ(Af[SET ^ 1][0], aa_, 0); FS2P_FENCE();                                                             \
        FS2P_WAIT_LGKM(4); FS2P_FENCE();                                                                                \
        FS2P_MFMA(SET, 0, 1, av0); FS2P_FENCE();                                                                        \
        FS2P_DS_READ(Bf[SET ^ 1][0], ba_, 0); FS2P_FENCE();                                                             \
        FS2P_WAIT_LGKM(4); FS2P_FENCE();                                                                                \
        FS2P_MFMA(SET, 0, 2, av0); FS2P_FENCE();                                                                        \
        FS2P_DS_READ(Bf[SET ^ 1][1], ba_, 4096); FS2P_FENCE();                                                          \
        FS2P_WAIT_LGKM(4); FS2P_FENCE();                                                                                \
        FS2P_MFMA(SET, 0, 3, av0); FS2P_FENCE();                                                                        \
        FS2P_DS_READ(Bf[SET ^ 1][2], ba_, 8192); FS2P_FENCE();                                                          \
        FS2P_WAIT_LGKM(4); FS2P_FENCE();                                                                                \
        av1 = Af[SET][1]; if (INACT) av1 = p_lrelu(av1, a.in_slope);                                                    \
        if (MASKED && !(LIVE1)) av1 = u32x4{0u, 0u, 0u, 0u};                                                            \
        FS2P_MFMA(SET, 1, 0, av1); FS2P_FENCE();                                                                        \
        FS2P_DS_READ(Bf[SET ^ 1][3], ba_, 12288); FS2P_FENCE();                                                         \
        FS2P_MFMA(SET, 1, 1, av1); FS2P_FENCE();                                                                        \
        FS2P_DS_READ(Af[SET ^ 1][1], aa_, 4096); FS2P_FENCE();                                                          \
        FS2P_MFMA(SET, 1, 2, av1); FS2P_FENCE();                                                                        \
        FS2P_MFMA(SET, 1, 3, av1); FS2P_FENCE();                                                                        \
    } while (0)

#define FS2P_SLICE1(SET, MASKED, LIVE0, JN, ABASE, AKEY, BBASE)                                                         \
    do {                                                                                                                \
        u32x4 av0;                                                                                                      \
        FS2P_WAIT_LGKM(3); FS2P_FENCE();                                                                                \
        av0 = Af[SET][0]; if (INACT) av0 = p_lrelu(av0, a.in_slope);                                                    \
        if (MASKED && !(LIVE0)) av0 = u32x4{0u, 0u, 0u, 0u};                                                            \
        FS2P_MFMA(SET, 0, 0, av0); FS2P_FENCE();                                                                        \
        const unsigned aa_ = (ABASE) + ((((AKEY)) ^ (unsigned)(JN)) << 4);                                              \
        const unsigned ba_ = (BBASE) + ((ckb ^ (unsigned)(JN)) << 4);                                                   \
        FS2P_DS_READ(Af[SET ^ 1][0], aa_, 0); FS2P_FENCE();                                                             \
        FS2P_WAIT_LGKM(3); FS2P_FENCE();                                                                                \
        FS2P_MFMA(SET, 0, 1, av0); FS2P_FENCE();                                                                        \
        FS2P_DS_READ(Bf[SET ^ 1][0], ba_, 0); FS2P_FENCE();                                                             \
        FS2P_WAIT_LGKM(3); FS2P_FENCE();                                                                                \
        FS2P_MFMA(SET, 0, 2, av0); FS2P_FENCE();                                                                        \
        FS2P_DS_READ(Bf[SET ^ 1][1], ba_, 4096); FS2P_FENCE();                                                          \
        FS2P_WAIT_LGKM(3); FS2P_FENCE();                                                                                \
        FS2P_MFMA(SET, 0, 3, av0); FS2P_FENCE();                                                                        \
        FS2P_DS_READ(Bf[SET ^ 1][2], ba_, 8192); FS2P_FENCE();                                                          \
        FS2P_DS_READ(Bf[SET ^ 1][3], ba_, 12288); FS2P_FENCE();                                                         \
    } while (0)
#define FS2P_SL(SET, MASKED, LIVE0, LIVE1, JN, ABASE, AKEY, BBASE)                                                      \
    do {                                                                                                                \
        if constexpr (MB == 2) { FS2P_SLICE(SET, MASKED, LIVE0, LIVE1, JN, ABASE, AKEY, BBASE); }                       \
        else { FS2P_SLICE1(SET, MASKED, LIVE0, JN, ABASE, AKEY, BBASE); }                                               \
    } while (0)

    auto land_set0 = [&]() {
        if constexpr (MB == 2)
            asm volatile("s_waitcnt lgkmcnt(0)" : "+v"(Af[0][0]), "+v"(Af[0][1]), "+v"(Bf[0][0]), "+v"(Bf[0][1]), "+v"(Bf[0][2]), "+v"(Bf[0][3]) :: "memory");
        else
            asm volatile("s_waitcnt lgkmcnt(0)" : "+v"(Af[0][0]), "+v"(Bf[0][0]), "+v"(Bf[0][1]), "+v"(Bf[0][2]), "+v"(Bf[0][3]) :: "memory");
    };
    int gs = 0, gc = 0, slot = 0;
    FS2P_WAIT_LGKM(0);
    __builtin_amdgcn_s_barrier();
    {
        const unsigned aa = a_base(0, 0) + (a_key(0) << 4), ba = b_base(0) + (ckb << 4);
        FS2P_DS_READ(Af[0][0], aa, 0); FS2P_DS_READ(Bf[0][0], ba, 0); FS2P_DS_READ(Bf[0][1], ba, 4096);
        FS2P_DS_READ(Bf[0][2], ba, 8192); FS2P_DS_READ(Bf[0][3], ba, 12288);
        if constexpr (MB == 2) FS2P_DS_READ(Af[0][1], aa, 4096);
        land_set0();
    }
    for (int k = 0; k < ntiles; ++k) {
        int mt, nt, kc0_unused;
        int split, nparts;
        p_tile_of(sc, k, units, mt, nt, kc0_unused, &split, &nparts);
        const int nkc_k = (k == ntiles - 1) ? nkc_last : nkc;
        const int m0 = mt * 256, n0 = nt * 128;
        unsigned vmask[2] = {0xffffffffu, 0xffffffffu};
        bool need_mask = false;
        if (!ONE_TAP) {
            const unsigned full = (taps >= 32) ? 0xffffffffu : ((1u << taps) - 1u);
#pragma unroll
            for (int mb = 0; mb < MB; ++mb) {
                const int m = m0 + wm * (32 * MB) + mb * 32 + fl;
                unsigned msk = 0;
                if (m < a.M) {
                    const int t = m % a.S;
                    for (int j = 0; j < taps; ++j) {
                        const int ts = t + j * a.dil - a.pad;
                        if (ts >= 0 && ts < a.S) msk |= 1u << j;
                    }
                }
                vmask[mb] = msk;
                need_mask = need_mask || (msk != full);
            }
            need_mask = __builtin_amdgcn_ballot_w64(need_mask) != 0ull;
        }
#pragma unroll
        for (int i = 0; i < MB; ++i)
#pragma unroll
            for (int j = 0; j < 4; ++j)
#pragma unroll
                for (int r = 0; r < 16; ++r) acc[i][j][r] = 0.f;

        auto run_tile = [&](auto maskc) {
            constexpr bool MASKED = decltype(maskc)::value;
            int tap = 0;
            for (int st = 0, nst = nkc_k * taps; st < nst; ++st) {
                {
                    const int abuf = ONE_TAP ? slot : (gc & 1);
                    const bool live0 = (vmask[0] >> tap) & 1u, live1 = (vmask[1] >> tap) & 1u;
                    const bool more = gs + 1 < total;
                    const unsigned ab = a_base(abuf, tap), ak = a_key(tap), bb = b_base(slot);
                    FS2P_SL(0, MASKED, live0, live1, 1, ab, ak, bb);
                    FS2P_SL(1, MASKED, live0, live1, 2, ab, ak, bb);
                    FS2P_SL(0, MASKED, live0, live1, 3, ab, ak, bb);
                    FS2P_WAIT_LGKM(0); FS2P_FENCE();
                    if (more) __builtin_amdgcn_s_barrier();
                    FS2P_FENCE();
                    int nslot = slot + 1; if (nslot == D) nslot = 0;
                    int ntap = tap + 1, ngc = gc; if (ntap == taps) { ntap = 0; ++ngc; }
                    const int nabuf = ONE_TAP ? nslot : (ngc & 1);
                    const unsigned nab = a_base(nabuf, ntap), nak = a_key(ntap), nbb = b_base(nslot);
                    FS2P_SL(1, MASKED, live0, live1, 0, nab, nak, nbb);
                    ++gs; slot = nslot; gc = ngc; tap = ntap;
                }
            }
        };
        if (need_mask) run_tile(std::true_type{}); else run_tile(std::false_type{});
        land_set0();

        if (nparts > 1) {
            p_epilogue_part(sc.tws + (size_t)sc.b * (256 * 128), acc, wm, fl, fh);
        } else if (sc.ks > 1) {
            p_epilogue_splitk(a, sc.ws + (size_t)split * a.M * a.N, acc, m0, n0, wm, fl, fh);
        } else {
            FS2_ACT_DISPATCH(a.act, (p_epilogue<ACT, MB>(a, acc, m0, n0, wm, fl, fh, lens_s, bias_s, lane)));
        }
    }
#undef FS2P_SL
#undef FS2P_SLICE1
#undef FS2P_SLICE
#undef FS2P_MFMA
}

template <bool ONE_TAP, bool WIDE, int INACT, int CW>
__global__ void __launch_bounds__(CW * 64 + 256, (CW + 4) / 4) conv_gemm_p_kernel(ConvGemmArgs a, PSched sc0) {
    extern __shared__ __attribute__((aligned(16))) unsigned char smem[];
    typedef PCfg<ONE_TAP, WIDE> C;
    const int tid = threadIdx.x, lane = tid & 63;
    const int wave = __builtin_amdgcn_readfirstlane(tid >> 6);
    PSched sc = sc0;
    sc.b = blockIdx.x;
    if (sc.tmap) {
        sc.n_real = __builtin_amdgcn_readfirstlane(sc.tmap[0]);
        sc.n_pad = sc.ntm - sc.n_real;
    }
    int32_t* lens_s = reinterpret_cast<int32_t*>(smem + C::AUX);
    float* bias_s = reinterpret_cast<float*>(smem + C::AUX + P_MAXB * 4) + (wave & 7) * 128;
    const int ntiles = p_ntiles(sc);
    PUnits units;
    p_units_load(sc, lane, units);
    if (wave < CW) {
        if (a.lens) {
            const int B = a.M / a.S;
            for (int i = tid; i < B; i += CW * 64) lens_s[i] = a.lens[i];
        }
        if (!a.accumulate && sc.n_pad > 0 && sc.ks == 1) {
            bf16_t* Y = reinterpret_cast<bf16_t*>(a.Y);
            const int n_pu = sc.n_pad * sc.ntn;
            for (int p = sc.b; p < n_pu; p += sc.G) {
                const int nt = p / sc.n_pad, pi = p - nt * sc.n_pad;
                const int m0 = sc.tmap[1 + sc.n_real + pi] * 256, n0 = nt * 128;
                for (int i = tid; i < 256 * 16; i += CW * 64) {
                    const int m = m0 + (i >> 4), n = n0 + (i & 15) * 8;
                    if (m < a.M && n < a.N) *reinterpret_cast<uint4*>(Y + (size_t)m * a.ldy + n) = make_uint4(0, 0, 0, 0);
                }
            }
        }
        if (ntiles > 0) p_consumer<ONE_TAP, WIDE, INACT, 8 / CW>(a, sc, smem, lane, wave, units, ntiles, lens_s, bias_s);
    } else if (ntiles > 0) {
        p_loader<ONE_TAP, WIDE>(a, sc, smem, lane, wave - CW, units, ntiles);
    }
}

__global__ void __launch_bounds__(64) tile_map_kernel(const int32_t* __restrict__ lens, int M, int S, int rows, int32_t* __restrict__ out) {
    const int lane = threadIdx.x;
    const int ntm = (M + rows - 1) / rows;
    int n_real = 0;
    for (int pass = 0; pass < 2; ++pass) {
        int n = 0;
        for (int base = 0; base < ntm; base += 64) {
            const int tm = base + lane;
            bool real = false, valid = tm < ntm;
            if (valid) {
                const int m0 = tm * rows, mlast = min(m0 + rows - 1, M - 1);
                const int b0 = m0 / S, b1 = mlast / S;
                real = !(b0 == b1 && (m0 - b0 * S) >= lens[b0]);
            }
            const bool pick = valid && (pass == 0 ? real : !real);
            const unsigned long long msk = __builtin_amdgcn_ballot_w64(pick);
            const int pos = n + __builtin_popcountll(msk & ((1ull << lane) - 1ull));
            if (pick) out[1 + (pass == 0 ? 0 : n_real) + pos] = tm;
            n += __builtin_popcountll(msk);
        }
        if (pass == 0) { n_real = n; if (lane == 0) out[0] = n; }
    }
}

__global__ void __launch_bounds__(256) lens_prep_kernel(const int64_t* __restrict__ lens, int B, int S, int rows,
                                                        int32_t* __restrict__ lens32, unsigned char* __restrict__ mask,
                                                        float* __restrict__ count, int32_t* __restrict__ tmap) {
    if (blockIdx.x > 0) {
        const long i0 = ((long)(blockIdx.x - 1) * 256 + threadIdx.x) * 4, n = (long)B * S;
        for (int e = 0; e < 4; ++e) {
            const long i = i0 + e;
            if (i < n) { const int b = (int)(i / S); mask[i] = (i - (long)b * S) >= lens[b]; }
        }
        return;
    }
    __shared__ int s_sum[4];
    int part = 0;
    for (int b = threadIdx.x; b < B; b += 256) {
        const long l = lens[b];
        const int v = (int)(l < 0 ? 0 : (l > S ? S : l));
        lens32[b] = v;
        part += v;
    }
    for (int o = 32; o > 0; o >>= 1) part += __shfl_xor(part, o, 64);
    if ((threadIdx.x & 63) == 0) s_sum[threadIdx.x >> 6] = part;
    __syncthreads();
    if (threadIdx.x == 0) count[0] = (float)(s_sum[0] + s_sum[1] + s_sum[2] + s_sum[3]);
    if (tmap && threadIdx.x < 64) {
        const int lane = threadIdx.x, M = B * S, ntm = (M + rows - 1) / rows;
        int n_real = 0;
        for (int pass = 0; pass < 2; ++pass) {
            int n = 0;
            for (int base = 0; base < ntm; base += 64) {
                const int tm = base + lane;
                bool real = false, valid = tm < ntm;
                if (valid) {
                    const int m0 = tm * rows, mlast = min(m0 + rows - 1, M - 1);
                    const int b0 = m0 / S, b1 = mlast / S;
                    real = !(b0 == b1 && (long)(m0 - b0 * S) >= lens[b0]);
                }
                const bool pick = valid && (pass == 0 ? real : !real);
                const unsigned long long msk = __builtin_amdgcn_ballot_w64(pick);
                const int pos = n + __builtin_popcountll(msk & ((1ull << lane) - 1ull));
                if (pick) tmap[1 + (pass == 0 ? 0 : n_real) + pos] = tm;
                n += __builtin_popcountll(msk);
            }
            if (pass == 0) { n_real = n; if (lane == 0) tmap[0] = n; }
        }
    }
}

extern "C" int fs2_lens_prep(const int64_t* lens, int B, int S, int rows, int32_t* lens32, void* mask, float* count,
                             int32_t* tile_map, hipStream_t stream) {
    FS2_CHECK_ARG(lens && lens32 && mask && count && B > 0 && S > 0 && rows > 0, "lens_prep: bad arguments");
    const long n = (long)B * S;
    lens_prep_kernel<<<1 + (unsigned)((n + 1023) / 1024), 256, 0, stream>>>(lens, B, S, rows, lens32, (unsigned char*)mask, count, tile_map);
    FS2_CHECK_LAUNCH("lens_prep");
    return FS2_OK;
}

extern "C" int fs2_tile_map(const int32_t* lens, int B, int S, int rows, int32_t* out, hipStream_t stream) {
    FS2_CHECK_ARG(lens && out && B > 0 && S > 0 && rows > 0, "tile_map: bad arguments");
    tile_map_kernel<<<1, 64, 0, stream>>>(lens, B * S, S, rows, out);
    FS2_CHECK_LAUNCH("tile_map");
    return FS2_OK;
}

static int fs2_cu_count() {
    static int cus[64] = {0};
    int d = 0;
    (void)hipGetDevice(&d);
    d &= 63;
    if (!cus[d]) {
        int n = 0;
        if (hipDeviceGetAttribute(&n, hipDeviceAttributeMultiprocessorCount, d) != hipSuccess || n <= 0) n = 256;
        cus[d] = n;
    }
    return cus[d];
}

template <bool ONE_TAP, bool WIDE, int INACT, int CW>
static void launch_p_cw(const ConvGemmArgs& a, const PSched& sc, hipStream_t stream) {
    constexpr int dyn = PCfg<ONE_TAP, WIDE>::AUX + P_AUX_BYTES;
    static Fs2DevOnce once;
    once.run([&] { (void)hipFuncSetAttribute((const void*)conv_gemm_p_kernel<ONE_TAP, WIDE, INACT, CW>, hipFuncAttributeMaxDynamicSharedMemorySize, dyn); });
    conv_gemm_p_kernel<ONE_TAP, WIDE, INACT, CW><<<(unsigned)sc.G, CW * 64 + 256, dyn, stream>>>(a, sc);
}
template <bool ONE_TAP, bool WIDE, int INACT>
static void launch_p(const ConvGemmArgs& a, const PSched& sc, hipStream_t stream) {
    if constexpr (!ONE_TAP && !WIDE) {
        if (a.N >= 1024) { launch_p_cw<ONE_TAP, WIDE, INACT, 8>(a, sc, stream); return; }
    }
    launch_p_cw<ONE_TAP, WIDE, INACT, 4>(a, sc, stream);
}

extern "C" int fs2_conv_gemm_tail_ws_bytes(void) { return fs2_cu_count() * 256 * 128 * (int)sizeof(float); }

bool fs2_conv_gemm_p_ok(const ConvGemmArgs& a, bool has_map, int dtype, int ks) {
    const bool inact = a.in_act == FS2_ACT_LRELU && a.in_slope > 0.f && a.in_slope < 1.f;
    if (dtype != FS2_BF16 || !(a.in_act == FS2_ACT_NONE || inact)) return false;
    const int taps = a.taps;
    if (!(taps == 1 || (taps >= 3 && (taps - 1) * a.dil <= 64 && taps <= 32))) return false;
    if (a.Cin % 64 != 0 || !a.vec_ok || a.N % 8 != 0) return false;
    if ((double)a.M * a.ldx * 2 >= 2.0e9 || (double)a.N * taps * a.Cin * 2 >= 2.0e9) return false;
    const long tiles = (long)fs2_cdiv(a.M, 256) * fs2_cdiv(a.N, 128) * ks;
    if (ks > 1 && ((a.Cin >> 6) % ks != 0 || a.accumulate)) return false;
    if (a.lens && (!has_map || a.M / a.S > P_MAXB)) return false;
    const int cus = fs2_cu_count();
    const bool long_conv = taps >= 3 && (long)taps * (a.Cin >> 6) >= 96 && tiles >= cus / 8;
    if (tiles < (ks > 1 ? cus / 4 : cus / 2) && !long_conv) return false;
    const long G = tiles < cus ? tiles : cus;
    const int ntm = fs2_cdiv(a.M, 256), ntn = fs2_cdiv(a.N, 128);
    if (ntn > 255) return false;
    if (p_max_units(ntm, ntn, ks, (int)G, 0) > 64 || (G % 8 == 0 && p_max_units(ntm, ntn, ks, (int)G, 1) > 64)) return false;
    return true;
}

void fs2_conv_gemm_p_launch(const ConvGemmArgs& a, const int32_t* tile_map, hipStream_t stream, int ks, float* ws, float* tail_ws) {
    const int ntm = fs2_cdiv(a.M, 256), ntn = fs2_cdiv(a.N, 128);
    const int cus = fs2_cu_count();
    PSched sc;
    sc.ks = ks; sc.nkc_u = (a.Cin >> 6) / ks; sc.ws = ws;
    sc.tws = nullptr; sc.tks_max = 1;
    if (tail_ws && ks == 1 && !a.accumulate && (long)ntm * ntn <= 2L * cus && (long)a.taps * sc.nkc_u >= 64) {
        int t = 1;
        while (t < 8 && sc.nkc_u % (2 * t) == 0 && a.taps * (sc.nkc_u / (2 * t)) >= 8) t *= 2;
        if (t >= 2) { sc.tws = tail_ws; sc.tks_max = t; }
    }
    sc.tmap = a.lens ? tile_map : nullptr;
    sc.ntm = ntm; sc.ntn = ntn; sc.b = 0;
    sc.n_real = ntm; sc.n_pad = 0;
    sc.G = (int)((long)ntm * ntn * ks < cus ? (long)ntm * ntn * ks : cus);
    if (sc.tws) sc.G = cus;
    const int taps = a.taps;
    sc.order = (ntn >= 2 && sc.G % 8 == 0 && (long)ntm * ntn * ks >= 2L * cus) ? 1 : 0;
    const bool wide = taps > 1 && (taps - 1) * a.dil > 16;
    if (a.in_act == FS2_ACT_LRELU) {
        if (taps == 1) launch_p<true, false, 1>(a, sc, stream);
        else if (wide) launch_p<false, true, 1>(a, sc, stream);
        else launch_p<false, false, 1>(a, sc, stream);
    } else if (taps == 1) launch_p<true, false, 0>(a, sc, stream);
    else if (wide) launch_p<false, true, 0>(a, sc, stream);
    else launch_p<false, false, 0>(a, sc, stream);
    if (ks > 1) {
        const long chunks = (long)a.M * (a.N >> 3);
        FS2_ACT_DISPATCH(a.act, (splitk_finalize_kernel<ACT><<<(unsigned)((chunks + 255) / 256), 256, 0, stream>>>(a, ws, ks)));
    }
    if (sc.tws) FS2_ACT_DISPATCH(a.act, (p_tail_finalize_kernel<ACT><<<dim3(4, (unsigned)((sc.G + 1) / 2)), 256, 0, stream>>>(a, sc)));
}
```

fastspeech2_amd/csrc/fs2_sched.h:

```cpp
#pragma once
#include <stdint.h>
#if defined(__HIPCC__)
#define FS2_HD __host__ __device__ __forceinline__
#else
#define FS2_HD inline
#endif

struct PSched {
    int G, b;
    int ntm, ntn;
    int n_real, n_pad;
    const int32_t* tmap;
    int ks, nkc_u;
    float* ws;
    float* tws;
    int tks_max;
    int order;
};

struct PPlan { int Gg, j, x, T, R, tail, tks; };
FS2_HD PPlan p_plan(const PSched& s, int b) {
    PPlan p;
    if (s.order == 0) { p.Gg = s.G; p.j = b; p.x = 0; p.T = s.n_real * s.ntn * s.ks; }
    else {
        p.x = b & 7; p.j = b >> 3; p.Gg = s.G >> 3;
        const int nx = s.n_real > p.x ? (s.n_real - p.x + 7) >> 3 : 0;
        p.T = nx * s.ntn * s.ks;
    }
    p.R = p.T / p.Gg;
    p.tail = p.T - p.R * p.Gg;
    p.tks = 1;
    if (s.tws && p.tail > 0) {
        int t = 1;
        while (2 * t <= s.tks_max && 2 * t * p.tail <= p.Gg) t *= 2;
        p.tks = t;
    }
    return p;
}
FS2_HD void p_pos(const PSched& s, const PPlan& p, int pos, int& mi, int& nt, int& sp) {
    if (s.order == 0) {
        const int rest = pos / s.ks;
        sp = pos - rest * s.ks;
        nt = rest / s.n_real;
        mi = rest - nt * s.n_real;
    } else {
        const int per = s.ntn * s.ks;
        const int mil = pos / per, r = pos - mil * per;
        nt = r / s.ks;
        sp = r - nt * s.ks;
        mi = p.x + 8 * mil;
    }
}
FS2_HD bool p_unit(const PSched& s, int k, int& mi, int& nt, int& kc0, int& nkc, int& np) {
    const PPlan p = p_plan(s, s.b);
    int pos, part = 0;
    np = 1;
    if (k < p.R) pos = k * p.Gg + p.j;
    else if (k == p.R && p.j < p.tail * p.tks) { pos = p.R * p.Gg + p.j / p.tks; part = p.j % p.tks; np = p.tks; }
    else return false;
    int sp;
    p_pos(s, p, pos, mi, nt, sp);
    nkc = s.nkc_u / np;
    kc0 = sp * s.nkc_u + part * nkc;
    return true;
}

FS2_HD int p_max_units(int n_real, int ntn, int ks, int G, int order) {
    long T, Gg;
    if (order == 0) { T = (long)n_real * ntn * ks; Gg = G; }
    else { T = (long)((n_real + 7) >> 3) * ntn * ks; Gg = G >> 3; }
    if (Gg <= 0) return 1 << 30;
    return (int)((T + Gg - 1) / Gg);
}

FS2_HD int fs2_tile_col128_bytes(int elem_bytes, int c) {
    if (elem_bytes != 2) return c;
    const int g = c >> 2, i = g >> 1;
    return (((g & 1) ? 16 + ((i + 4) & 15) : i) << 2) | (c & 3);
}
```

fastspeech2_amd/ops.py:

```python
import torch

from . import _lib

F32, BF16 = 0, 1
ACT_NONE, ACT_RELU, ACT_TANH, ACT_LRELU, ACT_GATE = 0, 1, 2, 3, 4

PROFILE = None


def dt(t_or_dtype):
    d = t_or_dtype.dtype if isinstance(t_or_dtype, torch.Tensor) else t_or_dtype
    if d == torch.float32:
        return F32
    if d == torch.bfloat16:
        return BF16
    raise TypeError(f"unsupported dtype {d}")


def _p(t):
    if t is None:
        return None
    assert t.is_cuda, "fs2 ops need device tensors (no CPU fallback)"
    return t.data_ptr()


_tls = __import__("threading").local()


def _stream():
    h = getattr(_tls, "handle", None)
    return h if h is not None else torch.cuda.current_stream().cuda_stream


class pinned_stream:

    def __init__(self, stream=None):
        self.stream = stream

    def __enter__(self):
        self.prev = getattr(_tls, "handle", None)
        s = self.stream if self.stream is not None else torch.cuda.current_stream()
        _tls.handle = s.cuda_stream
        return self

    def __exit__(self, *exc):
        _tls.handle = self.prev
        return False


def _contig(t):
    assert t.is_contiguous(), "fs2 ops need contiguous tensors"
    return t


def pack_weight(w, dtype, want_fwd=True, want_dgrad=True, wf=None, wd=None):
    w = _contig(w)
    if w.dim() == 2:
        cout, cin, k = w.shape[0], w.shape[1], 1
    else:
        cout, k, cin = w.shape
    if want_fwd and wf is None and dtype == torch.float32:
        wf, want_fwd_copy = w.view(cout, k, cin), False
    else:
        want_fwd_copy = want_fwd
    if want_fwd and wf is None:
        wf = torch.empty(cout, k, cin, device=w.device, dtype=dtype)
    if want_dgrad and wd is None:
        wd = torch.empty(cin, k, cout, device=w.device, dtype=dtype)
    if want_fwd_copy or want_dgrad:
        _lib.call("fs2_pack_weight", _p(w), _p(wf) if want_fwd_copy else None, _p(wd) if want_dgrad else None, cout, cin, k,
                  dt(dtype), _stream())
    return wf, wd


def conv_gemm(x, wpacked, bias, S, taps=1, dil=1, pad=0, act=ACT_NONE, slope=0.0, lens=None, res=None, out=None,
              in_act=ACT_NONE, in_slope=0.0, accumulate=False, out_scale=1.0, ldx=None, M=None, Cin=None, N=None,
              ldy=None, tmap=None, ksplit=1, ws=None, tail_ws=None, ragged=None, res_unlrelu=0.0, post_slope=0.0):
    if M is None:
        M = x.shape[0]
    if Cin is None:
        Cin = wpacked.shape[-1]
    if N is None:
        N = wpacked.shape[0]
    if ldx is None:
        ldx = x.stride(0)
    if out is None:
        out = torch.empty(M, N, device=x.device, dtype=x.dtype)
    if ldy is None:
        ldy = out.stride(0) if out.dim() == 2 else N
    ldr = res.stride(0) if res is not None else 0
    if PROFILE is not None:
        e0, e1 = torch.cuda.Event(enable_timing=True), torch.cuda.Event(enable_timing=True)
        e0.record()
    if res_unlrelu or post_slope:
        assert ksplit == 1 and lens is None and in_act == ACT_NONE
        _lib.call("fs2_conv_gemm_lrelu_io", _p(x), ldx, _p(wpacked), _p(bias), _p(res), ldr, _p(out), ldy, _p(tail_ws), M, N, Cin, S, taps,
                  dil, pad, act, slope, int(accumulate), out_scale, res_unlrelu, post_slope, dt(x), _stream())
    elif ksplit > 1:
        assert ws is not None and ws.numel() >= ksplit * M * N and ws.dtype == torch.float32 and in_act == ACT_NONE and not accumulate
        _lib.call("fs2_conv_gemm_splitk", _p(x), ldx, _p(wpacked), _p(bias), _p(res), ldr, _p(out), ldy, _p(lens), _p(tmap), _p(ws),
                  ksplit, M, N, Cin, S, taps, dil, pad, act, slope, out_scale, dt(x), _stream())
    elif tail_ws is not None:
        _lib.call("fs2_conv_gemm_tail", _p(x), ldx, _p(wpacked), _p(bias), _p(res), ldr, _p(out), ldy, _p(lens), _p(tmap), _p(tail_ws),
                  M, N, Cin, S, taps, dil, pad, act, slope, in_act, in_slope, int(accumulate), out_scale, dt(x), _stream())
    else:
        _lib.call("fs2_conv_gemm", _p(x), ldx, _p(wpacked), _p(bias), _p(res), ldr, _p(out), ldy, _p(lens), _p(tmap), M, N, Cin, S,
                  taps, dil, pad, act, slope, in_act, in_slope, int(accumulate), out_scale, dt(x), _stream())
    if PROFILE is not None:
        e1.record()
        if res_unlrelu or post_slope:
            var = _lib.load().fs2_conv_gemm_lrelu_io_variant(ldx, ldy, ldr, int(accumulate), M, N, Cin, S, taps, dil, act, res_unlrelu,
                                                             post_slope, dt(x))
        else:
            var = 5 if ksplit > 1 and taps > 1 else (6 if ksplit > 1 else
                  _lib.load().fs2_conv_gemm_variant(ldx, ldy, ldr, int(lens is not None), int(tmap is not None), M, N, Cin, S, taps, dil,
                                                    in_act, in_slope, dt(x)))
        PROFILE.setdefault("conv_gemm", []).append((2.0 * M * N * Cin * taps, e0, e1, var, (lens is not None) or bool(ragged), S))
    return out


def resblock_fwd(x, w1, w2, b1, b2, B, S, k, dilations, xs=None, out_scale=1.0, slope=0.1, post_slope=0.0):
    acc = xs is not None
    if xs is None:
        xs = torch.empty_like(x)
    d0, d1, d2 = dilations
    _lib.call("fs2_resblock_fwd", _p(x), x.stride(0), _p(w1), _p(w2), _p(b1), _p(b2), _p(xs), xs.stride(0), int(acc), out_scale, slope,
              post_slope, B, S, x.shape[1], k, d0, d1, d2, dt(x), _stream())
    return xs


def resstage_fwd(x, blocks, B, S, dilations, out_scale=1.0 / 3, slope=0.1, post_slope=0.0):
    xs = torch.empty_like(x)
    args = []
    for w1, w2, b1, b2, k in blocks:
        args += [_p(w1), _p(w2), _p(b1), _p(b2), k]
    d0, d1, d2 = dilations
    _lib.call("fs2_resstage_fwd", _p(x), x.stride(0), *args, _p(xs), xs.stride(0), out_scale, slope, post_slope, B, S, x.shape[1], d0, d1, d2,
              dt(x), _stream())
    return xs


def melgan_guard_rows(src, dst, G, reflect=True, interior=True):
    B, S, C = src.shape
    assert dst.shape == (B, S + 2 * G, C) and src.stride(2) == 1 and dst.stride(2) == 1 and src.dtype == dst.dtype
    _lib.call("fs2_melgan_guard_rows", _p(src), src.stride(1), src.stride(0), _p(dst), dst.stride(1), dst.stride(0), B, S, G, C,
              int(reflect), int(interior), dt(src), _stream())
    return dst


def melgan_stage_fwd(x, w, bias, y, dilations=(1, 3, 9), slope=0.2, out_slope=0.0):
    B, S, C = x.shape
    assert y.shape == x.shape and x.stride(2) == 1 and y.stride(2) == 1 and w.shape == (3, 5 * C, C) and w.is_contiguous()
    assert bias.shape == (3, 2, C) and bias.is_contiguous() and bias.dtype == torch.float32 and w.dtype == x.dtype == y.dtype
    d0, d1, d2 = dilations
    _lib.call("fs2_melgan_stage_fwd", _p(x), x.stride(1), x.stride(0), _p(w), _p(bias), _p(y), y.stride(1), y.stride(0), slope, out_slope,
              B, S, C, d0, d1, d2, dt(x), _stream())
    return y


def tail_workspace(device):
    return torch.empty(_lib.load().fs2_conv_gemm_tail_ws_bytes() // 4, device=device, dtype=torch.float32)


TILE_ROWS = 256


def lens_prep(lens, B, S, count_out):
    dev = lens.device
    lens = lens if (lens.dtype == torch.int64 and lens.is_contiguous()) else lens.to(torch.int64).contiguous()
    lens32 = torch.empty(B, device=dev, dtype=torch.int32)
    mask = torch.empty(B, S, device=dev, dtype=torch.bool)
    tmap = torch.empty(1 + (B * S + TILE_ROWS - 1) // TILE_ROWS, device=dev, dtype=torch.int32)
    _lib.call("fs2_lens_prep", _p(lens), B, S, TILE_ROWS, _p(lens32), _p(mask), _p(count_out), _p(tmap), _stream())
    return lens32, mask, tmap


def tile_map(lens, B, S):
    ntm = (B * S + TILE_ROWS - 1) // TILE_ROWS
    out = torch.empty(1 + ntm, device=lens.device, dtype=torch.int32)
    _lib.call("fs2_tile_map", _p(lens), B, S, TILE_ROWS, _p(out), _stream())
    return out


class WgradWorkspaces:

    def __init__(self):
        self._ws = {}
        self._retired = []

    def get(self, device, stream_handle, nbytes):
        key = (device.index, stream_handle)
        ws = self._ws.get(key)
        if ws is None or ws.numel() * 4 < nbytes:
            if ws is not None:
                self._retired.append(ws)
            ws = torch.empty(max(nbytes, _lib.load().fs2_conv_wgrad_ws_cap()) // 4 + 4, device=device, dtype=torch.float32)
            self._ws[key] = ws
        return ws

    def release_retired(self):
        self._retired.clear()


_default_wgrad_ws = WgradWorkspaces()


def wgrad_workspace(device, stream_handle, nbytes):
    return _default_wgrad_ws.get(device, stream_handle, nbytes)


def conv_wgrad(dy, x, dw, S, taps=1, dil=1, pad=0, lens=None, dbias=None, use_ws=True, ws_owner=None):
    M, N = dy.shape
    Cin = x.shape[1]
    if use_ws and dy.dtype == torch.bfloat16 and M > 0:
        need = _lib.load().fs2_conv_wgrad_ws_bytes(M, N, Cin, S, taps, dil, int(lens is not None), BF16)
        if need > 0:
            h = _stream()
            ws = (ws_owner or _default_wgrad_ws).get(dy.device, h, need)
            if PROFILE is not None:
                e0, e1 = torch.cuda.Event(enable_timing=True), torch.cuda.Event(enable_timing=True)
                e0.record()
            _lib.call("fs2_conv_wgrad_ws", _p(dy), dy.stride(0), _p(x), x.stride(0), _p(dw), _p(dbias), _p(lens), M, N, Cin, S, taps,
                      dil, pad, BF16, _p(ws), ws.numel() * 4, h)
            if PROFILE is not None:
                e1.record()
                PROFILE.setdefault("conv_wgrad", []).append((2.0 * M * N * Cin * taps, e0, e1, taps, lens is not None, S))
            return
    if PROFILE is not None:
        e0, e1 = torch.cuda.Event(enable_timing=True), torch.cuda.Event(enable_timing=True)
        e0.record()
    _lib.call("fs2_conv_wgrad", _p(dy), dy.stride(0), _p(x), x.stride(0), _p(dw), _p(dbias), _p(lens), M, N, Cin, S, taps, dil,
              pad, dt(dy), _stream())
    if PROFILE is not None:
        e1.record()
        PROFILE.setdefault("conv_wgrad", []).append((2.0 * M * N * Cin * taps, e0, e1, taps, lens is not None, S))


def colsum(x, out):
    M, N = x.shape
    _lib.call("fs2_colsum", _p(x), x.stride(0), _p(out), M, N, dt(x), _stream())


def attn_fwd(qkv, lens, B, S, H, dk=128):
    ctx = torch.empty(B * S, H * dk, device=qkv.device, dtype=qkv.dtype)
    lse = torch.empty(B, H, S, device=qkv.device, dtype=torch.float32)
    _lib.call("fs2_attn_fwd", _p(qkv), _p(ctx), _p(lse), _p(lens), B, S, H, dk, float(dk) ** -0.5, dt(qkv), _stream())
    return ctx, lse


def attn_bwd(qkv, ctx, dctx, lse, lens, B, S, H, dk=128):
    dqkv = torch.empty_like(qkv)
    delta = torch.empty_like(lse)
    _lib.call("fs2_attn_bwd", _p(qkv), _p(ctx), _p(dctx), _p(lse), _p(delta), _p(dqkv), _p(lens), B, S, H, dk,
              float(dk) ** -0.5, dt(qkv), _stream())
    return dqkv


def ln_fwd(y, res, gamma, beta, lens, B, S, eps=1e-5, p_pre=0.0, seed_pre=0, p_post=0.0, seed_post=0, seed_dev=None):
    C = y.shape[-1]
    out = torch.empty_like(y)
    mean = torch.empty(B * S, device=y.device, dtype=torch.float32)
    rstd = torch.empty(B * S, device=y.device, dtype=torch.float32)
    _lib.call("fs2_ln_fwd", _p(y), _p(res), _p(gamma), _p(beta), _p(lens), _p(out), _p(mean), _p(rstd), B, S, C, eps,
              p_pre, seed_pre, p_post, seed_post, _p(seed_dev), dt(y), _stream())
    return out, mean, rstd


def gemm_res_ln(x, wpacked, bias, res, gamma, beta, lens, tmap, B, S, eps=1e-5, p_pre=0.0, seed_pre=0, seed_dev=None, streaming_only=False):
    M, Cin = x.shape
    N = wpacked.shape[0]
    if x.dtype != torch.bfloat16 or wpacked.shape[1] != 1 or not _lib.load().fs2_gemm_res_ln_supported(M, N, Cin, S, BF16):
        return None
    streams = bool(_lib.load().fs2_gemm_res_ln_streams(M, N, Cin, S, BF16))
    if streaming_only and not streams:
        return None
    z = torch.empty(M, N, device=x.device, dtype=x.dtype)
    out = torch.empty(M, N, device=x.device, dtype=x.dtype)
    mean = torch.empty(M, device=x.device, dtype=torch.float32)
    rstd = torch.empty(M, device=x.device, dtype=torch.float32)
    if PROFILE is not None:
        e0, e1 = torch.cuda.Event(enable_timing=True), torch.cuda.Event(enable_timing=True)
        e0.record()
    _lib.call("fs2_gemm_res_ln_fwd", _p(x), x.stride(0), _p(wpacked), _p(bias), _p(res), res.stride(0) if res is not None else 0, _p(z), N,
              _p(out), N, _p(gamma), _p(beta), _p(mean), _p(rstd), _p(lens), _p(tmap), M, N, Cin, S, eps, p_pre, seed_pre, _p(seed_dev), BF16,
              _stream())
    if PROFILE is not None:
        e1.record()
        PROFILE.setdefault("conv_gemm", []).append((2.0 * M * N * Cin, e0, e1, 9 if streams else 7, lens is not None, S))
    return z, out, mean, rstd


def ln_bwd(z, dout, gamma, lens, mean, rstd, dgamma, dbeta, B, S, want_d1=True, want_d2=False, d1_add=None, p_pre=0.0,
           seed_pre=0, p_post=0.0, seed_post=0, relu_bwd=False, seed_dev=None, defer=False, dout2=None):
    C = z.shape[-1]
    d1 = torch.empty_like(z) if want_d1 else None
    d2 = torch.empty_like(z) if want_d2 else None
    ws = torch.empty(1024 * 2 * C + 4, device=z.device, dtype=torch.float32)
    _lib.call("fs2_ln_bwd_sum", _p(z), _p(dout), _p(dout2), _p(gamma), _p(lens), _p(mean), _p(rstd), _p(d1_add), _p(d1), _p(d2),
              _p(None if defer else dgamma), _p(None if defer else dbeta), _p(ws), B, S, C, p_pre, seed_pre, p_post, seed_post,
              _p(seed_dev), int(relu_bwd), dt(z), _stream())
    if defer:
        return d1, d2, ws
    return d1, d2


def ln_bwd_reduce(ws, C, dgamma, dbeta):
    _lib.call("fs2_ln_bwd_reduce", _p(ws), C, _p(dgamma), _p(dbeta), _stream())


def bn_apply_out32(x, mean_rstd, gamma, beta, res, act, p, seed, seed_dev=None, want_out=False, want_res32=True):
    M, C = x.shape
    out = torch.empty_like(x) if want_out else None
    out32 = torch.empty(M, C, device=x.device, dtype=torch.float32)
    res32 = torch.empty(M, C, device=x.device, dtype=torch.float32) if (want_res32 and res is not None) else None
    _lib.call("fs2_bn_apply_out32", _p(x), _p(mean_rstd), _p(gamma), _p(beta), _p(res), _p(out), _p(out32), _p(res32), M, C, act, p, seed,
              _p(seed_dev), dt(x), _stream())
    return out, out32, res32


def bn_train_fwd(x, gamma, beta, running_mean, running_var, act, p, seed, eps=1e-5, momentum=0.1, res=None, seed_dev=None,
                 ws=None, num_batches_tracked=None, out32=False):
    M, C = x.shape
    mean_rstd = torch.empty(2 * C, device=x.device, dtype=torch.float32)
    if ws is not None:
        _lib.call("fs2_bn_train_stats", _p(x), _p(ws), ws.numel(), _p(running_mean), _p(running_var), _p(num_batches_tracked), _p(mean_rstd),
                  M, C, eps, momentum, dt(x), _stream())
    else:
        stats = bn_workspace(C, x.device)
        _lib.call("fs2_bn_stats", _p(x), _p(stats), stats.numel(), M, C, dt(x), _stream())
        _lib.call("fs2_bn_finalize", _p(stats), _p(running_mean), _p(running_var), _p(mean_rstd), M, C, eps, momentum,
                  _stream())
    if out32:
        _, o32, r32 = bn_apply_out32(x, mean_rstd, gamma, beta, res, act, p, seed, seed_dev=seed_dev)
        return (o32, r32), mean_rstd
    out = torch.empty_like(x)
    _lib.call("fs2_bn_apply", _p(x), _p(mean_rstd), _p(gamma), _p(beta), _p(res), _p(out), M, C, act, p, seed, _p(seed_dev),
              dt(x), _stream())
    return out, mean_rstd


def bn_workspace(C, device):
    return torch.zeros(_lib.load().fs2_bn_ws_floats(C), device=device, dtype=torch.float32)


def bn_bwd_acc(x, dout, mean_rstd, gamma, beta, act, p, seed, ws, dgamma_acc, dbeta_acc, seed_dev=None):
    M, C = x.shape
    dx = torch.empty_like(x)
    _lib.call("fs2_bn_bwd_acc", _p(x), _p(dout), _p(mean_rstd), _p(gamma), _p(beta), _p(ws), ws.numel(), _p(dx), _p(dgamma_acc),
              _p(dbeta_acc), M, C, act, p, seed, _p(seed_dev), dt(x), _stream())
    return dx


def bn_bwd(x, dout, mean_rstd, gamma, beta, act, p, seed, seed_dev=None):
    M, C = x.shape
    sums = bn_workspace(C, x.device)
    dx = torch.empty_like(x)
    _lib.call("fs2_bn_bwd", _p(x), _p(dout), _p(mean_rstd), _p(gamma), _p(beta), _p(sums), sums.numel(), _p(dx), M, C, act, p, seed,
              _p(seed_dev), dt(x), _stream())
    return dx, sums[C:2 * C], sums[:C]


def embed_pe_fwd(tokens, emb, pe, dtype):
    B, L = tokens.shape
    V, C = emb.shape
    out = torch.empty(B * L, C, device=emb.device, dtype=dtype)
    _lib.call("fs2_embed_pe_fwd", _p(tokens), _p(emb), _p(pe), _p(out), B, L, C, V, dt(dtype), _stream())
    return out


def embed_bwd(tokens, dy, demb, pad_idx=0):
    V, C = demb.shape
    _lib.call("fs2_embed_bwd", _p(tokens), _p(dy), _p(demb), tokens.numel(), C, V, pad_idx, dt(dy), _stream())


def add_rowvec(x, table, idx, B, S):
    V, C = table.shape
    _lib.call("fs2_add_rowvec", _p(x), _p(table), _p(idx), B, S, C, V, dt(x), _stream())


def rowvec_bwd(dy, dtable, idx, B, S):
    V, C = dtable.shape
    _lib.call("fs2_rowvec_bwd", _p(dy), _p(dtable), _p(idx), B, S, C, V, dt(dy), _stream())


def bucket_embed_add_fwd(x, vals, scale, bins, emb):
    rows, C = x.shape
    out = torch.empty_like(x)
    idx = torch.empty(rows, device=x.device, dtype=torch.int32)
    _lib.call("fs2_bucket_embed_add_fwd", _p(x), _p(vals), float(scale), _p(bins), bins.numel(), _p(emb), _p(out),
              _p(idx), rows, C, dt(x), _stream())
    return out, idx


def bucket_embed_bwd(idx, dy, demb):
    rows, C = dy.shape
    _lib.call("fs2_bucket_embed_bwd", _p(idx), _p(dy), _p(demb), rows, demb.shape[0], C, dt(dy), _stream())


def lr_index(durations, T):
    B, L = durations.shape
    is_float = durations.dtype == torch.float32
    assert is_float or durations.dtype == torch.int64
    dev = durations.device
    cum = torch.empty(B, L + 1, device=dev, dtype=torch.int32)
    idx = torch.empty(B, T, device=dev, dtype=torch.int32)
    mel_len = torch.empty(B, device=dev, dtype=torch.int64)
    _lib.call("fs2_lr_index", _p(_contig(durations)), int(is_float), B, L, T, _p(cum), _p(idx), _p(mel_len), _stream())
    return cum, idx, mel_len


def lr_gather_fwd(x, idx, pe, B, L, T):
    C = x.shape[-1]
    out = torch.empty(B * T, C, device=x.device, dtype=x.dtype)
    _lib.call("fs2_lr_gather_fwd", _p(x), _p(idx), _p(pe), _p(out), B, L, T, C, dt(x), _stream())
    return out


def lr_gather_bwd(dy, cum, B, L, T, dx=None, accumulate=False):
    C = dy.shape[-1]
    if dx is None:
        dx = torch.empty(B * L, C, device=dy.device, dtype=dy.dtype)
    _lib.call("fs2_lr_gather_bwd", _p(dy), _p(cum), _p(dx), B, L, T, C, int(accumulate), dt(dy), _stream())
    return dx


def lr_gather_bwd_add(dy, cum, add1, add2, B, L, T):
    C = dy.shape[-1]
    dx0 = torch.empty(B * L, C, device=dy.device, dtype=dy.dtype)
    dx1 = torch.empty_like(dx0)
    dx2 = torch.empty_like(dx0) if add2 is not None else None
    _lib.call("fs2_lr_gather_bwd_add", _p(dy), _p(cum), _p(_contig(add1)), _p(add2), _p(dx0), _p(dx1), _p(dx2), B, L, T, C, dt(dy), _stream())
    return dx0, dx1, dx2


def duration_round(logd, d_control):
    out = torch.empty_like(logd)
    _lib.call("fs2_duration_round", _p(logd), float(d_control), _p(out), logd.numel(), _stream())
    return out


def rowdot_fwd(x, w, bias, lens, B, S):
    out = torch.empty(B, S, device=x.device, dtype=torch.float32)
    _lib.call("fs2_rowdot_fwd", _p(x), _p(w), _p(bias), _p(lens), _p(out), B, S, x.shape[-1], dt(x), _stream())
    return out


def rowdot_bwd(x, w, g, lens, dw, db, B, S):
    dx = torch.empty_like(x)
    _lib.call("fs2_rowdot_bwd", _p(x), _p(w), _p(g), _p(lens), _p(dx), _p(dw), _p(db), B, S, x.shape[-1], dt(x),
              _stream())
    return dx


def mask_rows(x, lens, B, S):
    _lib.call("fs2_mask_rows", _p(x), _p(lens), B, S, x.shape[-1], dt(x), _stream())
    return x


def cast(x, dtype, out=None):
    if out is None:
        out = torch.empty(x.shape, device=x.device, dtype=dtype)
    _lib.call("fs2_cast", _p(x), dt(x), _p(out), dt(dtype), x.numel(), _stream())
# ... 87 lines not shown
```

include/fs2hip.h:

```cpp
#ifndef FS2HIP_H
#define FS2HIP_H
#include <stddef.h>
#include <stdint.h>
#ifdef __cplusplus
extern "C" {
#endif

typedef struct ihipStream_t* fs2_stream_t;

enum { FS2_F32 = 0, FS2_BF16 = 1 };
enum { FS2_ACT_NONE = 0, FS2_ACT_RELU = 1, FS2_ACT_TANH = 2, FS2_ACT_LRELU = 3,
       FS2_ACT_GATE = 4  };

int fs2_version(void);
const char* fs2_last_error(void);

int fs2_conv_gemm(const void* X, long ldx, const void* Wpacked, const float* bias, const void* R, long ldr, void* Y,
                  long ldy, const int32_t* lens, const int32_t* tile_map, int M, int N, int Cin, int S, int taps, int dil,
                  int pad, int act, float slope, int in_act, float in_slope, int accumulate, float out_scale, int dtype,
                  fs2_stream_t stream);
int fs2_tile_map(const int32_t* lens, int B, int S, int rows, int32_t* out, fs2_stream_t stream);
int fs2_lens_prep(const int64_t* lens, int B, int S, int rows, int32_t* lens32, void* mask, float* count, int32_t* tile_map,
                  fs2_stream_t stream);
int fs2_conv_gemm_tail_ws_bytes(void);
int fs2_conv_gemm_tail(const void* X, long ldx, const void* Wpacked, const float* bias, const void* R, long ldr, void* Y,
                       long ldy, const int32_t* lens, const int32_t* tile_map, float* tail_ws, int M, int N, int Cin, int S,
                       int taps, int dil, int pad, int act, float slope, int in_act, float in_slope, int accumulate,
                       float out_scale, int dtype, fs2_stream_t stream);
int fs2_conv_gemm_splitk(const void* X, long ldx, const void* Wpacked, const float* bias, const void* R, long ldr, void* Y,
                         long ldy, const int32_t* lens, const int32_t* tile_map, float* ws, int ksplit, int M, int N, int Cin,
                         int S, int taps, int dil, int pad, int act, float slope, float out_scale, int dtype,
                         fs2_stream_t stream);
int fs2_conv_gemm_lrelu_io(const void* X, long ldx, const void* Wpacked, const float* bias, const void* R, long ldr, void* Y,
                           long ldy, float* tail_ws, int M, int N, int Cin, int S, int taps, int dil, int pad, int act, float slope,
                           int accumulate, float out_scale, float res_unlrelu, float post_slope, int dtype, fs2_stream_t stream);
int fs2_mfma_calibrate(int iters, float* sink, double* flops, fs2_stream_t stream);
int fs2_hbm_calibrate(const void* src, void* dst, size_t bytes, fs2_stream_t stream);
int fs2_ldsdma_calibrate(const void* src, size_t src_bytes, int iters, float* sink, double* bytes, fs2_stream_t stream);
#define FS2_GEMM_PLAIN 1
#define FS2_GEMM_DMA 2
#define FS2_GEMM_RING 3
#define FS2_GEMM_SKINNY 4
#define FS2_GEMM_PERSIST 5
#define FS2_GEMM_PERSIST_1TAP 6
#define FS2_GEMM_WIDE_1TAP 7
#define FS2_GEMM_STREAM_K256 9
int fs2_conv_gemm_variant(long ldx, long ldy, long ldr, int has_lens, int has_map, int M, int N, int Cin, int S, int taps,
                          int dil, int in_act, float in_slope, int dtype);
int fs2_conv_gemm_lrelu_io_variant(long ldx, long ldy, long ldr, int accumulate, int M, int N, int Cin, int S, int taps, int dil,
                                   int act, float res_unlrelu, float post_slope, int dtype);
int fs2_pack_weight(const float* w, void* wf, void* wd, int Cout, int Cin, int k, int dtype, fs2_stream_t stream);
int fs2_pack_dgrad_multi(const float* flat, void* wd_base, const int64_t* table, int n_entries, int total_tiles, int dtype,
                         fs2_stream_t stream);
int fs2_conv_wgrad(const void* dY, long lddy, const void* X, long ldx, float* dW, float* dbias, const int32_t* lens, int M,
                   int N, int Cin, int S, int taps, int dil, int pad, int dtype, fs2_stream_t stream);
int fs2_conv_wgrad_ws_bytes(int M, int N, int Cin, int S, int taps, int dil, int has_lens, int dtype);
int fs2_conv_wgrad_ws_cap(void);
int fs2_conv_wgrad_ws(const void* dY, long lddy, const void* X, long ldx, float* dW, float* dbias, const int32_t* lens, int M,
                      int N, int Cin, int S, int taps, int dil, int pad, int dtype, float* ws, long ws_bytes, fs2_stream_t stream);
int fs2_colsum(const void* x, long ldx, float* out, int M, int N, int dtype, fs2_stream_t stream);

int fs2_attn_fwd(const void* qkv, void* ctx, float* lse, const int32_t* lens, int B, int S, int H, int dk, float scale,
                 int dtype, fs2_stream_t stream);
int fs2_attn_bwd(const void* qkv, const void* ctx, const void* dctx, const float* lse, float* delta, void* dqkv,
                 const int32_t* lens, int B, int S, int H, int dk, float scale, int dtype, fs2_stream_t stream);

int fs2_ln_fwd(void* y, const void* res, const float* gamma, const float* beta, const int32_t* lens, void* out,
               float* mean, float* rstd, int B, int S, int C, float eps, float p_pre, uint64_t seed_pre, float p_post,
               uint64_t seed_post, const uint64_t* seed_dev, int dtype, fs2_stream_t stream);
int fs2_gemm_res_ln_supported(int M, int N, int Cin, int S, int dtype);
int fs2_gemm_res_ln_streams(int M, int N, int Cin, int S, int dtype);
int fs2_gemm_res_ln_fwd(const void* X, long ldx, const void* Wpacked, const float* bias, const void* R, long ldr, void* Z, long ldz,
                        void* out, long ldo, const float* gamma, const float* beta, float* mean, float* rstd, const int32_t* lens,
                        const int32_t* tile_map, int M, int N, int Cin, int S, float eps, float p_pre, uint64_t seed_pre,
                        const uint64_t* seed_dev, int dtype, fs2_stream_t stream);
#define FS2_LN_BWD_GRID 1024
int fs2_ln_bwd(const void* z, const void* dout, const float* gamma, const int32_t* lens, const float* mean,
               const float* rstd, const void* d1_add, void* d1, void* d2, float* dgamma, float* dbeta,
               float* partial_ws, int B, int S, int C, float p_pre, uint64_t seed_pre, float p_post, uint64_t seed_post, const uint64_t* seed_dev,
               int relu_bwd, int dtype, fs2_stream_t stream);
int fs2_ln_bwd_reduce(const float* partial_ws, int C, float* dgamma , float* dbeta , fs2_stream_t stream);
int fs2_ln_bwd_sum(const void* z, const void* dout, const void* dout2, const float* gamma, const int32_t* lens, const float* mean,
                   const float* rstd, const void* d1_add, void* d1, void* d2, float* dgamma, float* dbeta,
                   float* partial_ws, int B, int S, int C, float p_pre, uint64_t seed_pre, float p_post, uint64_t seed_post, const uint64_t* seed_dev,
                   int relu_bwd, int dtype, fs2_stream_t stream);

int fs2_bn_ws_floats(int C);
int fs2_bn_stats(const void* x, float* stats , long ws_floats, int M, int C,
                 int dtype, fs2_stream_t stream);
int fs2_bn_train_stats(const void* x, float* stats_ws, long ws_floats, float* running_mean, float* running_var,
                       int64_t* num_batches_tracked, float* mean_rstd, int M, int C, float eps, float momentum, int dtype,
                       fs2_stream_t stream);
int fs2_bn_finalize(const float* stats, float* running_mean, float* running_var, float* mean_rstd , int M, int C,
                    float eps, float momentum, fs2_stream_t stream);
int fs2_bn_apply(const void* x, const float* mean_rstd, const float* gamma, const float* beta, const void* res, void* out,
                 int M, int C, int act, float p, uint64_t seed, const uint64_t* seed_dev, int dtype, fs2_stream_t stream);
int fs2_bn_apply_out32(const void* x, const float* mean_rstd, const float* gamma, const float* beta, const void* res, void* out,
                       float* out32, float* res32, int M, int C, int act, float p, uint64_t seed, const uint64_t* seed_dev,
                       int dtype, fs2_stream_t stream);
int fs2_bn_bwd(const void* x, const void* dout, const float* mean_rstd, const float* gamma, const float* beta,
               float* sums , long ws_floats, void* dx, int M, int C, int act, float p,
               uint64_t seed, const uint64_t* seed_dev, int dtype, fs2_stream_t stream);
int fs2_bn_bwd_acc(const void* x, const void* dout, const float* mean_rstd, const float* gamma, const float* beta, float* sums,
                   long ws_floats, void* dx, float* dgamma_acc, float* dbeta_acc, int M, int C, int act, float p, uint64_t seed,
                   const uint64_t* seed_dev, int dtype, fs2_stream_t stream);

int fs2_embed_pe_fwd(const int64_t* tokens, const float* emb, const float* pe, void* out, int B, int L, int C, int V,
                     int dtype, fs2_stream_t stream);
int fs2_embed_bwd(const int64_t* tokens, const void* dy, float* demb, int rows, int C, int V, int pad_idx, int dtype,
                  fs2_stream_t stream);
int fs2_add_rowvec(void* x, const float* table, const int64_t* idx, int B, int S, int C, int V, int dtype,
                   fs2_stream_t stream);
int fs2_rowvec_bwd(const void* dy, float* dtable, const int64_t* idx, int B, int S, int C, int V, int dtype,
                   fs2_stream_t stream);
int fs2_bucket_embed_add_fwd(const void* x, const float* vals, float scale, const float* bins, int nbins,
                             const float* emb, void* out, int32_t* idx_out, int rows, int C, int dtype,
                             fs2_stream_t stream);
int fs2_bucket_embed_bwd(const int32_t* idx, const void* dy, float* demb, int rows, int n_bins, int C, int dtype,
                         fs2_stream_t stream);
int fs2_lr_index(const void* durations, int dur_is_float, int B, int L, int T, int32_t* cum, int32_t* idx,
                 int64_t* mel_len, fs2_stream_t stream);
int fs2_lr_gather_fwd(const void* x, const int32_t* idx, const float* pe, void* out, int B, int L, int T, int C,
                      int dtype, fs2_stream_t stream);
int fs2_lr_gather_bwd(const void* dy, const int32_t* cum, void* dx, int B, int L, int T, int C, int accumulate,
                      int dtype, fs2_stream_t stream);
int fs2_lr_gather_bwd_add(const void* dy, const int32_t* cum, const void* add1, const void* add2, void* dx0, void* dx1, void* dx2,
                          int B, int L, int T, int C, int dtype, fs2_stream_t stream);
int fs2_duration_round(const float* logd, float d_control, float* out, int n, fs2_stream_t stream);
int fs2_rowdot_fwd(const void* x, const float* w, const float* bias, const int32_t* lens, float* out, int B, int S, int C,
                   int dtype, fs2_stream_t stream);
int fs2_rowdot_bwd(const void* x, const float* w, const float* g, const int32_t* lens, void* dx, float* dw, float* db,
                   int B, int S, int C, int dtype, fs2_stream_t stream);
int fs2_mask_rows(void* x, const int32_t* lens, int B, int S, int C, int dtype, fs2_stream_t stream);
int fs2_cast(const void* in, int in_dtype, void* out, int out_dtype, size_t n, fs2_stream_t stream);
int fs2_add(const void* a, const void* b, void* out, size_t n, int dtype, fs2_stream_t stream);
int fs2_add_pe(void* x, const float* pe, int B, int S, int C, int dtype, fs2_stream_t stream);
int fs2_bump_counter(uint64_t* ctr, uint64_t inc, fs2_stream_t stream);

int fs2_chan_to_rows(const float* in, void* out, int B, int C, int T, int dtype, fs2_stream_t stream);
int fs2_conv_post_pcm(const void* x, long ldx, const float* w, const float* bias, float in_slope, float* wav,
                      int16_t* pcm, float max_wav_value, int M, int S, int C, int taps, int pad, int dtype,
                      fs2_stream_t stream);
int fs2_resblock_supported(int C, int k, int d0, int d1, int d2, int dtype);
int fs2_resblock_fwd(const void* x, long ldx, const void* w1, const void* w2, const float* b1, const float* b2, void* xs,
                     long ldxs, int accumulate, float out_scale, float slope, float post_slope, int B, int S, int C, int k, int d0,
                     int d1, int d2, int dtype, fs2_stream_t stream);
int fs2_resstage_fwd(const void* x, long ldx, const void* w1a, const void* w2a, const float* b1a, const float* b2a, int ka,
                     const void* w1b, const void* w2b, const float* b1b, const float* b2b, int kb, const void* w1c,
                     const void* w2c, const float* b1c, const float* b2c, int kc, void* xs, long ldxs, float out_scale,
                     float slope, float post_slope, int B, int S, int C, int d0, int d1, int d2, int dtype, fs2_stream_t stream);
int fs2_melgan_guard_rows(const void* src, long ld_src, long src_bstride, void* dst, long ld_dst, long dst_bstride, int B, int S,
                          int G, int C, int reflect, int interior, int dtype, fs2_stream_t stream);
int fs2_melgan_stage_supported(int C, int dtype);
int fs2_melgan_stage_fwd(const void* x, long ldx, long x_bstride, const void* w, const float* bias, void* y, long ldy, long y_bstride,
                         float slope, float out_slope, int B, int S, int C, int d0, int d1, int d2, int dtype, fs2_stream_t stream);
int fs2_reflect_pad(const float* y, float* xp, int B, int N, int P, long row_len, fs2_stream_t stream);
int fs2_reflect_pad_ragged(const float* y, long ldy, const int32_t* lens, float* xp, int B, int P, long row_len,
                           fs2_stream_t stream);
int fs2_stft_mel_epilogue(const float* ft, long ldft, const float* mel_basis, const int32_t* span, float* mel,
                          float* energy, int B, int S, int frames, int NF, int n_mel, float clamp_min,
                          fs2_stream_t stream);

int fs2_gl_mel_to_mag(const float* mel, long sb, long sj, long st, const int32_t* mel_lens, const float* mel_basis,
                      const int32_t* span, float* mag, long ldm, int B, int Fmax, int n_mel, int NF, fs2_stream_t stream);
int fs2_gl_recombine(const float* mag, long msb, long msf, long msk, const float* phase, long psb, long psf, long psk,
                     const int32_t* frames, float* G, long ldg, int B, int Fmax, int NF, fs2_stream_t stream);
int fs2_gl_project(const float* ft, long ldft, int S, const float* mag, long msb, long msf, long msk, const int32_t* frames,
                   float* G, long ldg, int B, int Fmax, int NF, fs2_stream_t stream);
int fs2_gl_ola(const float* seg, long lds, const int32_t* frames, const double* win_sq, float* xp, long row_len, float* y,
               long ldy, int B, int Fmax, int filter_length, int hop_length, fs2_stream_t stream);
int fs2_gl_mag_phase(const float* ft, long ldft, int S, float* mag, float* phase, int B, int F, int NF, fs2_stream_t stream);

int fs2_resample_poly(const float* x, long ldx, const int32_t* in_begin, const int32_t* in_len, const double* tab, int up,
                      int down, int half, int T, const int32_t* out_begin, const int32_t* out_len, float* y, float* yc, long ldy,
                      int B, int Nin, int Nout, fs2_stream_t stream);
int fs2_peak_abs(const float* y, long ldy, const int32_t* lens, float* peak, int B, int Nmax, fs2_stream_t stream);
int fs2_peaknorm_pcm(const float* y, long ldy, const int32_t* lens, const float* peak, float max_wav_value, int16_t* pcm, long ldp,
                     int B, int Nmax, fs2_stream_t stream);

int fs2_f0_dc(const float* x, long ldx, const int32_t* lens, double* stats, int B, int Nmax, fs2_stream_t stream);
int fs2_f0_lowcut(const float* x, long ldx, const int32_t* lens, const double* stats, const double* taps, int R, double* lc,
                  long ldl, int H, int B, int Nmax, fs2_stream_t stream);
int fs2_f0_events(const double* lc, long ldl, int H, const int32_t* lens, const double* stats, const double* nuttall,
                  const int32_t* band_h, int nb, int max_h, int32_t* counts, const int32_t* offs, double* events, long cap, int B,
                  int Nmax, int emit, fs2_stream_t stream);
int fs2_f0_scan(const int32_t* counts, int32_t* offs, int32_t* totals, int B, int nb, int Nmax, fs2_stream_t stream);
int fs2_f0_candidates(const double* events, long cap, const int32_t* totals, const int32_t* frames, const double* band_f0,
                      int nb, double fs, double frame_period, double f0_floor, double f0_ceil, double* cand, double* score,
                      int B, int Fmax, fs2_stream_t stream);
int fs2_f0_fix(const double* cand, const double* score, const int32_t* frames, int nb, int vrm, double allowed_range,
               double* tmp, double* f0, int B, int Fmax, fs2_stream_t stream);
int fs2_f0_stonemask(const float* x, long ldx, const int32_t* lens, const double* f0, const int32_t* frames, double fs,
                     double frame_period, double* out, int B, int Fmax, int Nmax, fs2_stream_t stream);

int fs2_pyin_cmnd(const float* x, long ldx, const int32_t* lens, const int32_t* frames, int hop, int frame_length, int tmax,
                  double* dprime, int B, int Fmax, int Nmax, fs2_stream_t stream);
int fs2_pyin_observe(const double* dprime, const int32_t* frames, int tmin, int tmax, const double* beta, int nthr,
                     double no_trough_prob, double fs, double fmin, int bins_per_octave, int nb, double* obs, double* pv,
                     int B, int Fmax, fs2_stream_t stream);
int fs2_pyin_viterbi(const double* obs, const int32_t* frames, int nb, int half_width, const double* logw, const double* logz,
                     double switch_prob, double fmin, int bins_per_octave, uint8_t* backptr, int32_t* states, double* f0,
                     int B, int Fmax, fs2_stream_t stream);

int fs2_align_max_states(void);
int fs2_align_feats(const float* mel, long ldm_b, long ldm_c, const int32_t* lens, double* mean, double* x, long ldx_b, long ldx_t,
                    int B, int n_mel, int Tmax, fs2_stream_t stream);
int fs2_align_emit(const double* x, long ldx_b, long ldx_t, const int32_t* lens, const int32_t* jlens, const int32_t* sid, long ldg,
                   const double* mu, const double* var, int n_classes, int D, double* E, long lde_b, long lde_t, int B, int Tmax,
                   int Jmax, fs2_stream_t stream);
int fs2_align_max_mixtures(void);
int fs2_align_emit_gmm(const double* x, long ldx_b, long ldx_t, const int32_t* lens, const int32_t* jlens, const int32_t* sid, long ldg,
                       const double* w, const double* mu, const double* var, int n_classes, int M, int D, double* E, long lde_b,
                       long lde_t, double* resp, long ldr_b, long ldr_t, long ldr_j, int B, int Tmax, int Jmax, fs2_stream_t stream);
int fs2_align_forward(const double* E, long lde_b, long lde_t, const int32_t* lens, const int32_t* jlens, const int32_t* skip,
                      long ldg, const int32_t* alt, double* alpha, long lda_b, long lda_t, double* loglik, int B, int Tmax, int Jmax,
                      fs2_stream_t stream);
int fs2_align_backward(const double* E, long lde_b, long lde_t, const int32_t* lens, const int32_t* jlens, const int32_t* skip,
                       long ldg, const int32_t* alt, const double* alpha, long lda_b, long lda_t, const double* loglik, double* gamma,
                       long ldo_b, long ldo_t, int B, int Tmax, int Jmax, fs2_stream_t stream);
int fs2_align_stats(const double* gamma, long ldo_b, long ldo_t, const double* x, long ldx_b, long ldx_t, const int32_t* lens,
                    const int32_t* jlens, int D, double* partials, long ldp_b, long ldp_j, int B, int Tmax, int Jmax,
                    fs2_stream_t stream);
int fs2_align_stats_gmm(const double* gamma, long ldo_b, long ldo_t, const double* resp, long ldr_b, long ldr_t, long ldr_j,
                        const double* x, long ldx_b, long ldx_t, const int32_t* lens, const int32_t* jlens, int M, int D,
                        double* partials, long ldp_b, long ldp_r, int B, int Tmax, int Jmax, fs2_stream_t stream);
int fs2_align_reduce(const double* partials, long ldp_j, long n_rows, const int32_t* offs, const int32_t* items, int n_classes,
                     int cols, double* sums, int accumulate, fs2_stream_t stream);
int fs2_align_viterbi(const double* E, long lde_b, long lde_t, const int32_t* lens, const int32_t* jlens, const int32_t* skip,
                      long ldg, const int32_t* alt, uint8_t* bp, long ldp_b, long ldp_t, int32_t* end, double* score, int B, int Tmax,
                      int Jmax, fs2_stream_t stream);
int fs2_align_backtrack(const uint8_t* bp, long ldp_b, long ldp_t, const int32_t* lens, const int32_t* jlens, const int32_t* skip,
                        const int32_t* block, long ldg, const int32_t* end, int32_t* frames, int nbmax, int B, int Tmax, int Jmax,
                        fs2_stream_t stream);
int fs2_align_max_splice_dim(void);
int fs2_align_splice(const double* x, long ldx_b, long ldx_t, const int32_t* lens, int n_mel, int c, double* y, long ldy_b, long ldy_t,
                     int B, int Tmax, fs2_stream_t stream);
int fs2_align_scatter_ws(int B, int Tmax, int Ds);
int fs2_align_scatter(const double* y, long ldy_b, long ldy_t, const int32_t* lens, int Ds, double* s, double* S, long lds, double* ws,
                      long ws_doubles, int B, int Tmax, fs2_stream_t stream);
int fs2_align_project(const double* y, long ldy_b, long ldy_t, const int32_t* lens, const double* P, const double* o, int K, int Ds,
                      double* z, long ldz_b, long ldz_t, int B, int Tmax, fs2_stream_t stream);
int fs2_align_max_fmllr_dim(void);
int fs2_align_fmllr_weights(const double* gamma, long ldg_b, long ldg_t, const int32_t* lens, const int32_t* jlens, const int32_t* sid,
                            long ldsid, const double* mu, const double* var, int n_classes, int D, double* c, double* h, long ldc_b,
                            long ldc_t, int B, int Tmax, int Jmax, fs2_stream_t stream);
int fs2_align_fmllr_accum_ws(int B, int Tmax, int D);
int fs2_align_fmllr_accum(const double* f, long ldf_b, long ldf_t, const double* c, const double* h, long ldc_b, long ldc_t,
                          const int32_t* lens, const int32_t* offs, const int32_t* rows, int n_spk, int D, double* beta, double* G,
                          double* k, double* ws, long ws_doubles, int B, int Tmax, fs2_stream_t stream);
int fs2_align_fmllr_apply(const double* f, long ldf_b, long ldf_t, const int32_t* lens, const double* W, const int32_t* spk, int n_spk,
                          int D, double* out, long ldo_b, long ldo_t, int B, int Tmax, fs2_stream_t stream);
int fs2_align_max_tree_sets(void);
int fs2_align_tree_gains(const double* sums, long lds, int n_items, const int32_t* left, const int32_t* right, const int32_t* offs,
                         const int32_t* items, int n_list, int n_nodes, const uint8_t* member, int n_sets, int n_symbols,
                         const double* floor, int D, double min_occ, int32_t* best_q, double* best_gain, double* gains, double* n_yes,
                         long ldq, fs2_stream_t stream);

int fs2_dtw_max_frames(void);
int fs2_mcep(const float* mel, long ldm_b, long ldm_c, const int32_t* lens, const double* table, int K, double* c, long ldc_b,
             long ldc_t, int B, int n_mel, int Tmax, fs2_stream_t stream);
int fs2_dtw_cost(const double* a, long lda_b, long lda_t, const int32_t* alens, const double* b, long ldb_b, long ldb_t,
                 const int32_t* blens, int K, double* cost, long ldd_b, long ldd_s, int B, int T1max, int T2max, fs2_stream_t stream);
int fs2_dtw_scan(const double* cost, long ldd_b, long ldd_s, const int32_t* alens, const int32_t* blens, uint8_t* bp, long ldp_b,
                 long ldp_s, double* total, int B, int T1max, int T2max, fs2_stream_t stream);
int fs2_dtw_backtrack(const uint8_t* bp, long ldp_b, long ldp_s, const int32_t* alens, const int32_t* blens, int32_t* pi, int32_t* pj,
                      long ldq, int32_t* plen, int B, int T1max, int T2max, fs2_stream_t stream);
int fs2_dtw_f0(const int32_t* pi, const int32_t* pj, long ldq, const int32_t* plen, const double* f0_ref, long ldr,
               const double* f0_syn, long lds, const int32_t* alens, const int32_t* blens, double* sums, long ldo, int B, int T1max,
               int T2max, fs2_stream_t stream);
int fs2_dtw_prosody(const int32_t* pi, const int32_t* pj, long ldq, const int32_t* plen, const double* f0_ref, long ldr,
                    const double* f0_syn, long lds, const float* e_ref, long lder, const float* e_syn, long ldes, const int32_t* alens,
                    const int32_t* blens, double* sums, long ldo, int B, int T1max, int T2max, fs2_stream_t stream);
int fs2_prosody_voiced(const double* f0, long ldf, const int32_t* lens, double* out, long ldo, int32_t* nv, double* stats, long lds,
                       int B, int Tmax, fs2_stream_t stream);

int fs2_env_spectrum(const float* x, long ldx, const int32_t* lens, const double* f0, long ldf, const int32_t* frames, double fs,
                     double frame_period, const double* twiddle, int N, double* P, long ldp_b, long ldp_t, int B, int Fmax, int Nmax,
                     fs2_stream_t stream);
int fs2_env_smooth(const double* f0, long ldf, const int32_t* frames, double fs, const double* twiddle, int N, double q1,
                   double env_floor, double* P, long ldp_b, long ldp_t, int B, int Fmax, fs2_stream_t stream);
int fs2_env_mcep(const double* env, long lde_b, long lde_t, const int32_t* frames, const double* twiddle, int N, const double* table,
                 int K, double* c, long ldc_b, long ldc_t, int B, int Fmax, fs2_stream_t stream);

int fs2_loss_fwd(const float* mel, const float* post, const float* mel_t, long ld_t_b, const int64_t* mel_lens,
                 const int64_t* src_lens, const float* p_pred, const float* p_t, long ld_pt, const float* e_pred,
                 const float* e_t, long ld_et, const float* logd, const int64_t* dur, long ld_dur, const float* cnt,
                 int B, int T, int L, int n_mel, int p_frame, int e_frame, float* sums, float* losses, fs2_stream_t stream);
int fs2_loss_bwd(const float* mel, const float* post, const float* mel_t, long ld_t_b, const int64_t* mel_lens,
                 const int64_t* src_lens, const float* p_pred, const float* p_t, long ld_pt, const float* e_pred,
                 const float* e_t, long ld_et, const float* logd, const int64_t* dur, long ld_dur, const float* cnt,
                 const float* g, int B, int T, int L, int n_mel, int p_frame, int e_frame, float* dmel, float* dpost,
                 float* dp, float* de, float* dlogd, fs2_stream_t stream);
int fs2_loss_fwd_ws(const float* mel, const float* post, const float* mel_t, long ld_t_b, const int64_t* mel_lens,
                    const int64_t* src_lens, const float* p_pred, const float* p_t, long ld_pt, const float* e_pred,
                    const float* e_t, long ld_et, const float* logd, const int64_t* dur, long ld_dur, const float* cnt,
                    int B, int T, int L, int n_mel, int p_frame, int e_frame, float* sums_ws, float* losses, fs2_stream_t stream);
int fs2_loss_bwd_lp(const float* mel, const float* post, const float* mel_t, long ld_t_b, const int64_t* mel_lens,
                    const int64_t* src_lens, const float* p_pred, const float* p_t, long ld_pt, const float* e_pred,
                    const float* e_t, long ld_et, const float* logd, const int64_t* dur, long ld_dur, const float* cnt,
                    const float* g_total, const float* g_mel, const float* g_post, const float* g_pitch, const float* g_energy,
                    const float* g_dur, int B, int T, int L, int n_mel, int p_frame, int e_frame, void* dmel, void* dpost,
                    int grad_dtype, float* dp, float* de, float* dlogd, fs2_stream_t stream);

#define FS2_SUMSQ_BLOCKS 1024
int fs2_sumsq(const float* x, size_t n, float* out , float* ws, fs2_stream_t stream);
int fs2_sumsq_set(const float* x, size_t n, float* out , float* ws, fs2_stream_t stream);
int fs2_adam_step(float* p, float* g, float* m, float* v, size_t n, const float* gnorm_sq, float max_norm,
                  const float* hyper, float b1, float b2, float eps, float wd, void* p_lowp, int lowp_dtype, int zero_grad,
                  fs2_stream_t stream);
int fs2_adam_step_h(float* p, float* g, float* m, float* v, size_t n, const float* gnorm_sq, float max_norm, float lr, float bc1,
                    float bc2, float b1, float b2, float eps, float wd, void* p_lowp, int lowp_dtype, int zero_grad,
                    fs2_stream_t stream);

#ifdef __cplusplus
}
#endif
#endif
```

include/fs2hip_testaid.h:

```cpp
#ifndef FS2HIP_TESTAID_H
#define FS2HIP_TESTAID_H
#ifdef __cplusplus
extern "C" {
#endif
int fs2t_stage_tile_col(int c, int elem_bytes);
int fs2t_conv_gemm_p_units(int n_real, int ntn, int G, int order, int ks, int nkc, int tks_max, int b, int* out, int max_units);
int fs2t_conv_gemm_p_max_units(int n_real, int ntn, int ks, int G, int order);
#ifdef __cplusplus
}
#endif
#endif
```

Before: 4.691 million mel-frames/s.

## Add dynamic atomic tile handout queue to persistent conv GEMM

Replaces the persistent GEMM's per-lane precomputed unit list with a small LDS ring queue that consumer wave 0 refills as tiles finish. Refills come either from a global atomic counter (dynamic handout) or from the static schedule, and the loader and consumer now stop on a zero-nkc sentinel instead of a precomputed tile count. Dynamic mode is compiled off by default (FS2_P_AUTO_DYNAMIC=0), so the default path still uses the static order through the new queue machinery. The queue adds LDS traffic, extra barriers and a tile-map copy into LDS.

```diff
diff --git a/fastspeech2_amd/csrc/fs2_common.h b/fastspeech2_amd/csrc/fs2_common.h
--- a/fastspeech2_amd/csrc/fs2_common.h
+++ b/fastspeech2_amd/csrc/fs2_common.h
@@ -121,4 +121,9 @@
 #define FS2_GEMM_WIDE_1TAP 7
 #define FS2_GEMM_STREAM_K256 9
 #endif
+#ifndef FS2_HANDOUT_AUTO
+#define FS2_HANDOUT_AUTO (-1)
+#define FS2_HANDOUT_STATIC 0
+#define FS2_HANDOUT_DYNAMIC 1
+#endif
 static inline int fs2_cdiv(long a, long b) { return (int)((a + b - 1) / b); }
diff --git a/fastspeech2_amd/csrc/fs2_gemm.hip b/fastspeech2_amd/csrc/fs2_gemm.hip
--- a/fastspeech2_amd/csrc/fs2_gemm.hip
+++ b/fastspeech2_amd/csrc/fs2_gemm.hip
@@ -823,7 +823,8 @@
 bool fs2_conv_gemm_w_ok(const ConvGemmArgs& a, bool has_map, int dtype);
 void fs2_conv_gemm_w_launch(const ConvGemmArgs& a, const int32_t* tile_map, hipStream_t stream);
 bool fs2_conv_gemm_p_ok(const ConvGemmArgs& a, bool has_map, int dtype, int ks);
-void fs2_conv_gemm_p_launch(const ConvGemmArgs& a, const int32_t* tile_map, hipStream_t stream, int ks, float* ws, float* tail_ws);
+void fs2_conv_gemm_p_launch(const ConvGemmArgs& a, const int32_t* tile_map, hipStream_t stream, int ks, float* ws, float* tail_ws,
+                            int handout);
 
 bool fs2_conv_gemm_s_ok(const ConvGemmArgs& a, int dtype);
 void fs2_conv_gemm_s_launch(const ConvGemmArgs& a, hipStream_t stream);
@@ -907,7 +908,7 @@
     } else if (pk.variant == FS2_GEMM_WIDE_1TAP) {
         fs2_conv_gemm_w_launch(a, tile_map, stream);
     } else if (pk.variant == FS2_GEMM_PERSIST || pk.variant == FS2_GEMM_PERSIST_1TAP) {
-        fs2_conv_gemm_p_launch(a, tile_map, stream, 1, nullptr, tail_ws);
+        fs2_conv_gemm_p_launch(a, tile_map, stream, 1, nullptr, tail_ws, FS2_HANDOUT_AUTO);
     } else if (pk.variant == FS2_GEMM_RING) {
         static Fs2DevOnce ring_once;
         const int dyn1 = RingCfg<true>::B_OFF + RingCfg<true>::D * RING_B_BYTES;
@@ -976,8 +977,25 @@
     ConvGemmArgs a;
     conv_gemm_fill(a, X, ldx, W, bias, R, ldr, Y, ldy, lens, M, N, Cin, S, taps, dil, pad, act, slope, FS2_ACT_NONE, 0.f, 0, out_scale, dtype);
     FS2_CHECK_ARG(fs2_conv_gemm_p_ok(a, tile_map != nullptr, dtype, ksplit), "conv_gemm_splitk: shape not supported (M=%d N=%d Cin=%d taps=%d ksplit=%d)", M, N, Cin, taps, ksplit);
-    fs2_conv_gemm_p_launch(a, tile_map, stream, ksplit, ws, nullptr);
+    fs2_conv_gemm_p_launch(a, tile_map, stream, ksplit, ws, nullptr, FS2_HANDOUT_AUTO);
     FS2_CHECK_LAUNCH("conv_gemm_splitk");
+    return FS2_OK;
+}
+
+extern "C" int fs2_conv_gemm_p(const void* X, long ldx, const void* W, const float* bias, const void* R, long ldr, void* Y, long ldy,
+                               const int32_t* lens, const int32_t* tile_map, float* tail_ws, float* ws, int ksplit, int handout, int M,
+                               int N, int Cin, int S, int taps, int dil, int pad, int act, float slope, int accumulate,
+                               float out_scale, int dtype, hipStream_t stream) {
+    FS2_CHECK_ARG(X && W && Y && (ksplit == 1 || (ksplit >= 2 && ws)), "conv_gemm_p: null pointer");
+    FS2_CHECK_ARG(M > 0 && N > 0 && Cin > 0 && S > 0 && taps > 0 && dil > 0 && M % S == 0, "conv_gemm_p: bad shape");
+    FS2_CHECK_ARG(handout >= FS2_HANDOUT_AUTO && handout <= FS2_HANDOUT_DYNAMIC, "conv_gemm_p: handout %d", handout);
+    FS2_CHECK_ARG(((uintptr_t)X & 15) == 0 && ((uintptr_t)W & 15) == 0 && ((uintptr_t)ws & 15) == 0 && ((uintptr_t)tail_ws & 15) == 0 && ldx % 8 == 0,
+                  "conv_gemm_p: alignment");
+    ConvGemmArgs a;
+    conv_gemm_fill(a, X, ldx, W, bias, R, ldr, Y, ldy, lens, M, N, Cin, S, taps, dil, pad, act, slope, FS2_ACT_NONE, 0.f, accumulate, out_scale, dtype);
+    FS2_CHECK_ARG(fs2_conv_gemm_p_ok(a, tile_map != nullptr, dtype, ksplit), "conv_gemm_p: shape not supported (M=%d N=%d Cin=%d taps=%d ksplit=%d)", M, N, Cin, taps, ksplit);
+    fs2_conv_gemm_p_launch(a, tile_map, stream, ksplit, ksplit > 1 ? ws : nullptr, ksplit > 1 ? nullptr : tail_ws, handout);
+    FS2_CHECK_LAUNCH("conv_gemm_p");
     return FS2_OK;
 }
 
diff --git a/fastspeech2_amd/csrc/fs2_gemm_p.hip b/fastspeech2_amd/csrc/fs2_gemm_p.hip
--- a/fastspeech2_amd/csrc/fs2_gemm_p.hip
+++ b/fastspeech2_amd/csrc/fs2_gemm_p.hip
@@ -23,52 +23,48 @@
 }
 template <int N> __device__ __forceinline__ void p_wait_vm() { asm volatile("s_waitcnt vmcnt(%0)" :: "n"(N) : "memory"); }
 static constexpr int P_MAXB = 1024;
-static constexpr int P_AUX_BYTES = P_MAXB * 4 + 8 * 512;
+static constexpr int P_QN = 8;
+static constexpr int P_TMAP_MAX = 512;
+static constexpr int P_Q_OFF = P_MAXB * 4 + 8 * 512;
+static constexpr int P_TMAP_OFF = P_Q_OFF + P_QN * 8;
+static constexpr int P_AUX_BYTES = P_TMAP_OFF + P_TMAP_MAX * 4;
 static constexpr int P_B_BYTES = 128 * 128;
 
-__device__ __forceinline__ int p_ntiles(const PSched& s) {
-    const PPlan p = p_plan(s, s.b);
-    return p.R + (p.j < p.tail * p.tks ? 1 : 0);
-}
-__device__ __forceinline__ int p_last_nkc(const PSched& s) {
-    const PPlan p = p_plan(s, s.b);
-    return (p.j < p.tail * p.tks) ? s.nkc_u / p.tks : s.nkc_u;
-}
-
-struct PUnits { unsigned v0, v1; };
-__device__ __forceinline__ void p_units_load(const PSched& s, int lane, PUnits& t) {
+typedef __attribute__((address_space(3))) volatile unsigned p_lds_vu;
+__device__ __forceinline__ p_lds_vu* p_lds(void* q) { return (p_lds_vu*)(__attribute__((address_space(3))) void*)q; }
+__device__ __forceinline__ int p_q_read(const PSched& s, unsigned* q, int k, int& mt, int& nt, int& kc0, int* split = nullptr,
+                                        int* nparts = nullptr) {
+    p_lds_vu* e = p_lds(q) + 2 * (k & (P_QN - 1));
+    const unsigned a0 = __builtin_amdgcn_readfirstlane(e[0]), a1 = __builtin_amdgcn_readfirstlane(e[1]);
+    mt = (int)(a0 & 0xfffffu);
+    nt = (int)((a0 >> 20) & 0xffu);
+    kc0 = (int)(a1 & 0xffffu);
+    if (nparts) *nparts = (int)(a0 >> 28);
+    if (split) *split = kc0 / s.nkc_u;
+    return (int)(a1 >> 16);
+}
+__device__ __forceinline__ int p_q_nkc(unsigned* q, int k) {
+    return (int)(__builtin_amdgcn_readfirstlane(p_lds(q)[2 * (k & (P_QN - 1)) + 1]) >> 16);
+}
+__device__ __forceinline__ void p_entry(const PSched& s, const PPlan& p, int pos, bool tail_turn, const int32_t* tmap_s,
+                                        unsigned& a0, unsigned& a1) {
     int mi, nt, kc0, nkc, np;
-    unsigned a0 = 0, a1 = 0;
-    if (p_unit(s, lane, mi, nt, kc0, nkc, np)) {
-        const int mt = s.tmap ? s.tmap[1 + mi] : mi;
+    a0 = 0; a1 = 0;
+    if (p_unit_at(s, p, pos, tail_turn, mi, nt, kc0, nkc, np)) {
+        const int mt = s.tmap ? (tmap_s ? tmap_s[mi] : s.tmap[1 + mi]) : mi;
         a0 = (unsigned)mt | ((unsigned)nt << 20) | ((unsigned)np << 28);
         a1 = (unsigned)kc0 | ((unsigned)nkc << 16);
     }
-    t.v0 = a0; t.v1 = a1;
-}
-__device__ __forceinline__ void p_tile_of(const PSched& s, int k, const PUnits& t, int& mt, int& nt, int& kc0, int* split = nullptr,
-                                          int* nparts = nullptr) {
-    const unsigned a0 = __builtin_amdgcn_readlane(t.v0, k), a1 = __builtin_amdgcn_readlane(t.v1, k);
-    mt = (int)(a0 & 0xfffffu);
-    nt = (int)((a0 >> 20) & 0xffu);
-    kc0 = __builtin_amdgcn_readfirstlane((int)(a1 & 0xffffu));
-    if (nparts) *nparts = (int)(a0 >> 28);
-    if (split) *split = kc0 / s.nkc_u;
-}
+}
+struct PClaimer { int kn; bool done; };
 
 template <bool ONE_TAP, bool WIDE>
-__device__ __forceinline__ void p_loader(const ConvGemmArgs& a, const PSched& sc, unsigned char* smem, int lane, int lw,
-                                         const PUnits& units, int ntiles) {
+__device__ __forceinline__ void p_loader(const ConvGemmArgs& a, const PSched& sc, unsigned char* smem, int lane, int lw, unsigned* q) {
     typedef PCfg<ONE_TAP, WIDE> C;
     constexpr int D = C::D, NJA = C::NJA;
     const unsigned char* Xb = reinterpret_cast<const unsigned char*>(a.X);
     const unsigned char* Wb = reinterpret_cast<const unsigned char*>(a.W);
-    const int nkc = sc.nkc_u;
-    const int nkc_last = p_last_nkc(sc);
     const int taps = ONE_TAP ? 1 : a.taps;
-    const int nsteps = taps * nkc;
-    const int total = (ntiles - 1) * nsteps + taps * nkc_last;
-    const int nchunks = (ntiles - 1) * nkc + nkc_last;
     int kc0A = 0, kc0B = 0;
     const int lr = lane >> 3, lc = lane & 7;
     const int arows = 256 + (taps - 1) * a.dil;
@@ -77,7 +73,7 @@
     unsigned offA[NJA], ldsA[NJA], offB[4];
     auto set_A = [&](int k) {
         int mt, nt;
-        p_tile_of(sc, k, units, mt, nt, kc0A);
+        p_q_read(sc, q, k, mt, nt, kc0A);
         const int m0 = mt * 256;
 #pragma unroll
         for (int j = 0; j < NJA; ++j) {
@@ -91,7 +87,7 @@
     };
     auto set_B = [&](int k) {
         int mt, nt;
-        p_tile_of(sc, k, units, mt, nt, kc0B);
+        p_q_read(sc, q, k, mt, nt, kc0B);
         const int n0 = nt * 128;
 #pragma unroll
         for (int j = 0; j < 4; ++j) {
@@ -100,7 +96,8 @@
             offB[j] = (unsigned)n * (unsigned)(a.ldw * 2) + (unsigned)((lc ^ ((r >> 1) & 7)) << 4);
         }
     };
-    int is = 0, ik = 0, ikc = 0, itap = 0, islot = 0;
+    int ik = 0, ikc = 0, itap = 0, islot = 0;
+    int i_nkc = p_q_nkc(q, 0), isd = 0;
     int kA = -1, kB = -1;
     auto issue_A = [&](int k, int kc, int buf_or_slot) {
         if (k != kA) { set_A(k); kA = k; }
@@ -112,45 +109,46 @@
         }
     };
     auto issue_step = [&]() {
+        if (i_nkc < 0) i_nkc = p_q_nkc(q, ik);
+        if (i_nkc == 0) return;
         if (ik != kB) { set_B(ik); kB = ik; }
         if (ONE_TAP) issue_A(ik, ikc, islot);
         const unsigned char* base = p_uniform(Wb + ((size_t)itap * a.Cin + (size_t)(kc0B + ikc) * 64) * 2);
         const unsigned d0 = smem_base + C::B_OFF + islot * P_B_BYTES + lw * 4096;
 #pragma unroll
         for (int j = 0; j < 4; ++j) glds16_sbase(offB[j], base, d0 + j * 1024);
-    };
-    auto advance_issue = [&]() {
-        ++is;
-        if (++itap == taps) { itap = 0; if (++ikc == (ik == ntiles - 1 ? nkc_last : nkc)) { ikc = 0; ++ik; } }
+        ++isd;
+        if (++itap == taps) { itap = 0; if (++ikc == i_nkc) { ikc = 0; ++ik; i_nkc = -1; } }
         if (++islot == D) islot = 0;
     };
     if (!ONE_TAP) issue_A(0, 0, 0);
 #pragma unroll
-    for (int p = 0; p < D - 1; ++p) {
-        if (is < total) issue_step();
-        advance_issue();
-    }
+    for (int p = 0; p < D - 1; ++p) issue_step();
     int ck = 0, ckc = 0, ctap = 0, gc = 0;
-    for (int cs = 0; cs < total; ++cs) {
-        if (total - 1 - cs < D - 2) {
+    int c_nkc = p_q_nkc(q, 0);
+    bool halo = false;
+    for (int cs = 0; c_nkc > 0; ++cs) {
+        if (isd - 1 - cs < D - 2) {
             asm volatile("s_waitcnt vmcnt(0)" ::: "memory");
         } else if (ONE_TAP) {
             p_wait_vm<(D - 2) * (NJA + 4)>();
         } else {
-            const bool a_young = (ctap >= 1 && ctap <= D - 2) && (gc + 1 < nchunks);
+            const bool a_young = (ctap >= 1 && ctap <= D - 2) && halo;
             if (a_young) p_wait_vm<(D - 2) * 4 + NJA>();
             else p_wait_vm<(D - 2) * 4>();
         }
         __builtin_amdgcn_s_barrier();
-        if (!ONE_TAP && ctap == 0 && gc + 1 < nchunks) {
+        asm volatile("" ::: "memory");
+        if (!ONE_TAP && ctap == 0) {
             int nk = ck, nkc_ = ckc + 1;
-            if (nkc_ == (ck == ntiles - 1 ? nkc_last : nkc)) { nkc_ = 0; ++nk; }
-            issue_A(nk, nkc_, (gc + 1) & 1);
-        }
-        if (is < total) issue_step();
-        advance_issue();
-        if (++ctap == taps) { ctap = 0; ++gc; if (++ckc == (ck == ntiles - 1 ? nkc_last : nkc)) { ckc = 0; ++ck; } }
-    }
+            halo = true;
+            if (nkc_ == c_nkc) { nkc_ = 0; ++nk; halo = p_q_nkc(q, nk) > 0; }
+            if (halo) issue_A(nk, nkc_, (gc + 1) & 1);
+        }
+        issue_step();
+        if (++ctap == taps) { ctap = 0; ++gc; if (++ckc == c_nkc) { ckc = 0; ++ck; c_nkc = p_q_nkc(q, ck); } }
+    }
+    __builtin_amdgcn_s_barrier();
 }
 
 #define FS2P_DS_READ(dst, addr, OFF) asm volatile("ds_read_b128 %0, %1 offset:" #OFF : "=v"(dst) : "v"(addr))
@@ -321,15 +319,13 @@
 }
 
 template <bool ONE_TAP, bool WIDE, int INACT, int MB>
-__device__ __forceinline__ void p_consumer(const ConvGemmArgs& a, const PSched& sc, unsigned char* smem, int lane, int wm,
-                                           const PUnits& units, int ntiles, const int32_t* lens_s, float* bias_s) {
+__device__ __forceinline__ void p_consumer(const ConvGemmArgs& a, const PSched& sc, const PPlan& pl, unsigned char* smem, int lane,
+                                           int wm, unsigned* q, PClaimer cl, const int32_t* tmap_s, const int32_t* lens_s,
+                                           float* bias_s) {
     typedef PCfg<ONE_TAP, WIDE> C;
     constexpr int D = C::D;
-    const int nkc = sc.nkc_u;
-    const int nkc_last = p_last_nkc(sc);
     const int taps = ONE_TAP ? 1 : a.taps;
-    const int nsteps = taps * nkc;
-    const int total = (ntiles - 1) * nsteps + taps * nkc_last;
+    int32_t* const cnt = sc.cnt ? sc.cnt + (sc.order ? pl.x : 0) : nullptr;
     const int fl = lane & 31, fh = lane >> 5;
     const unsigned smem_u = lds_addr(smem);
     const unsigned c0 = (unsigned)(fh * 4);
@@ -409,7 +405,7 @@
         else
             asm volatile("s_waitcnt lgkmcnt(0)" : "+v"(Af[0][0]), "+v"(Bf[0][0]), "+v"(Bf[0][1]), "+v"(Bf[0][2]), "+v"(Bf[0][3]) :: "memory");
     };
-    int gs = 0, gc = 0, slot = 0;
+    int gc = 0, slot = 0;
     FS2P_WAIT_LGKM(0);
     __builtin_amdgcn_s_barrier();
     {
@@ -419,11 +415,11 @@
         if constexpr (MB == 2) FS2P_DS_READ(Af[0][1], aa, 4096);
         land_set0();
     }
-    for (int k = 0; k < ntiles; ++k) {
+    for (int k = 0;; ++k) {
         int mt, nt, kc0_unused;
         int split, nparts;
-        p_tile_of(sc, k, units, mt, nt, kc0_unused, &split, &nparts);
-        const int nkc_k = (k == ntiles - 1) ? nkc_last : nkc;
+        const int nkc_k = p_q_read(sc, q, k, mt, nt, kc0_unused, &split, &nparts);
+        if (nkc_k == 0) break;
         const int m0 = mt * 256, n0 = nt * 128;
         unsigned vmask[2] = {0xffffffffu, 0xffffffffu};
         bool need_mask = false;
@@ -455,36 +451,53 @@
         auto run_tile = [&](auto maskc) {
             constexpr bool MASKED = decltype(maskc)::value;
             int tap = 0;
-            for (int st = 0, nst = nkc_k * taps; st < nst; ++st) {
+            int st = 0;
+            const int nst = nkc_k * taps;
+            do {
                 {
                     const int abuf = ONE_TAP ? slot : (gc & 1);
                     const bool live0 = (vmask[0] >> tap) & 1u, live1 = (vmask[1] >> tap) & 1u;
-                    const bool more = gs + 1 < total;
                     const unsigned ab = a_base(abuf, tap), ak = a_key(tap), bb = b_base(slot);
                     FS2P_SL(0, MASKED, live0, live1, 1, ab, ak, bb);
                     FS2P_SL(1, MASKED, live0, live1, 2, ab, ak, bb);
                     FS2P_SL(0, MASKED, live0, live1, 3, ab, ak, bb);
                     FS2P_WAIT_LGKM(0); FS2P_FENCE();
-                    if (more) __builtin_amdgcn_s_barrier();
+                    __builtin_amdgcn_s_barrier();
                     FS2P_FENCE();
                     int nslot = slot + 1; if (nslot == D) nslot = 0;
                     int ntap = tap + 1, ngc = gc; if (ntap == taps) { ntap = 0; ++ngc; }
                     const int nabuf = ONE_TAP ? nslot : (ngc & 1);
                     const unsigned nab = a_base(nabuf, ntap), nak = a_key(ntap), nbb = b_base(nslot);
                     FS2P_SL(1, MASKED, live0, live1, 0, nab, nak, nbb);
-                    ++gs; slot = nslot; gc = ngc; tap = ntap;
+                    slot = nslot; gc = ngc; tap = ntap;
                 }
-            }
+            } while (++st < nst);
+            land_set0();
         };
         if (need_mask) run_tile(std::true_type{}); else run_tile(std::false_type{});
         land_set0();
 
+        const bool claiming = wm == 0 && !cl.done;
+        int cv = 0;
+        if (claiming && cnt && lane == 0) cv = atomicAdd(cnt, 1);
         if (nparts > 1) {
             p_epilogue_part(sc.tws + (size_t)sc.b * (256 * 128), acc, wm, fl, fh);
         } else if (sc.ks > 1) {
             p_epilogue_splitk(a, sc.ws + (size_t)split * a.M * a.N, acc, m0, n0, wm, fl, fh);
         } else {
             FS2_ACT_DISPATCH(a.act, (p_epilogue<ACT, MB>(a, acc, m0, n0, wm, fl, fh, lens_s, bias_s, lane)));
+        }
+        if (claiming) {
+            const int pos = cnt ? __builtin_amdgcn_readfirstlane(cv) : p_static_pos(pl, cl.kn);
+            unsigned a0, a1;
+            p_entry(sc, pl, pos, true, tmap_s, a0, a1);
+            cl.done = pos >= pl.R * pl.Gg;
+            if (lane == 0) {
+                p_lds_vu* e = p_lds(q);
+                e[2 * (cl.kn & (P_QN - 1))] = a0; e[2 * (cl.kn & (P_QN - 1)) + 1] = a1;
+                if (cl.done) e[2 * ((cl.kn + 1) & (P_QN - 1)) + 1] = 0u;
+            }
+            ++cl.kn;
         }
     }
 #undef FS2P_SL
@@ -507,13 +520,40 @@
     }
     int32_t* lens_s = reinterpret_cast<int32_t*>(smem + C::AUX);
     float* bias_s = reinterpret_cast<float*>(smem + C::AUX + P_MAXB * 4) + (wave & 7) * 128;
-    const int ntiles = p_ntiles(sc);
-    PUnits units;
-    p_units_load(sc, lane, units);
+    unsigned* q = reinterpret_cast<unsigned*>(smem + C::AUX + P_Q_OFF);
+    int32_t* tmap_s = (sc.tmap && sc.ntm <= P_TMAP_MAX) ? reinterpret_cast<int32_t*>(smem + C::AUX + P_TMAP_OFF) : nullptr;
+    const PPlan pl = p_plan(sc, sc.b);
+    PClaimer cl = {0, true};
+    if (wave == 0) {
+        int pos0 = 0;
+        if (sc.cnt) {
+            int v = 0;
+            if (lane == 0) v = atomicAdd(sc.cnt + (sc.order ? pl.x : 0), sc.la + 1);
+            pos0 = __builtin_amdgcn_readfirstlane(v);
+        }
+        const int lim = pl.R * pl.Gg;
+        const int it = sc.cnt ? max(lim - pos0, 0) : pl.R;
+        const int pos = sc.cnt ? pos0 + lane : p_static_pos(pl, lane);
+        unsigned a0, a1;
+        p_entry(sc, pl, pos, lane == it, nullptr, a0, a1);
+        if (lane <= sc.la || (lane == sc.la + 1 && it <= sc.la)) {
+            p_lds_vu* e = p_lds(q);
+            e[2 * lane] = a0; e[2 * lane + 1] = a1;
+        }
+        cl.kn = sc.la + 1;
+        cl.done = it <= sc.la;
+        asm volatile("s_waitcnt lgkmcnt(0)" ::: "memory");
+    }
+    __builtin_amdgcn_s_barrier();
+    asm volatile("" ::: "memory");
+    const bool any = p_q_nkc(q, 0) > 0;
     if (wave < CW) {
         if (a.lens) {
             const int B = a.M / a.S;
             for (int i = tid; i < B; i += CW * 64) lens_s[i] = a.lens[i];
+        }
+        if (tmap_s && any) {
+            for (int i = tid; i < sc.ntm; i += CW * 64) tmap_s[i] = sc.tmap[1 + i];
         }
         if (!a.accumulate && sc.n_pad > 0 && sc.ks == 1) {
             bf16_t* Y = reinterpret_cast<bf16_t*>(a.Y);
@@ -527,9 +567,14 @@
                 }
             }
         }
-        if (ntiles > 0) p_consumer<ONE_TAP, WIDE, INACT, 8 / CW>(a, sc, smem, lane, wave, units, ntiles, lens_s, bias_s);
-    } else if (ntiles > 0) {
-        p_loader<ONE_TAP, WIDE>(a, sc, smem, lane, wave - CW, units, ntiles);
+        if (any) p_consumer<ONE_TAP, WIDE, INACT, 8 / CW>(a, sc, pl, smem, lane, wave, q, cl, tmap_s, lens_s, bias_s);
+        if (sc.cnt && tid == 0) {
+            if (atomicAdd(sc.cnt + 8, 1) == sc.G - 1) {
+                for (int i = 0; i <= 8; ++i) atomicExch(sc.cnt + i, 0);
+            }
+        }
+    } else if (any) {
+        p_loader<ONE_TAP, WIDE>(a, sc, smem, lane, wave - CW, q);
     }
 }
 
@@ -670,7 +715,34 @@
     return true;
 }
 
-void fs2_conv_gemm_p_launch(const ConvGemmArgs& a, const int32_t* tile_map, hipStream_t stream, int ks, float* ws, float* tail_ws) {
+#ifndef FS2_P_AUTO_DYNAMIC
+#define FS2_P_AUTO_DYNAMIC 0
+#endif
+static constexpr bool P_AUTO_DYNAMIC = FS2_P_AUTO_DYNAMIC != 0;
+static constexpr int P_SLOTS = 1024;
+extern "C" int fs2_conv_gemm_p_slots(void) { return P_SLOTS; }
+static int32_t* p_slot_next(hipStream_t stream) {
+    static int32_t* ring[64] = {nullptr};
+    static unsigned next[64] = {0};
+    static std::mutex mu;
+    int d = 0;
+    (void)hipGetDevice(&d);
+    d &= 63;
+    std::lock_guard<std::mutex> g(mu);
+    if (!ring[d]) {
+        hipStreamCaptureStatus st = hipStreamCaptureStatusNone;
+        if (hipStreamIsCapturing(stream, &st) != hipSuccess || st != hipStreamCaptureStatusNone) return nullptr;
+        void* p = nullptr;
+        const size_t bytes = (size_t)P_SLOTS * P_SLOT_WORDS * sizeof(int32_t);
+        if (hipMalloc(&p, bytes) != hipSuccess) return nullptr;
+        if (hipMemset(p, 0, bytes) != hipSuccess || hipDeviceSynchronize() != hipSuccess) { (void)hipFree(p); return nullptr; }
+        ring[d] = static_cast<int32_t*>(p);
+    }
+    return ring[d] + (size_t)(next[d]++ % P_SLOTS) * P_SLOT_WORDS;
+}
+
+void fs2_conv_gemm_p_launch(const ConvGemmArgs& a, const int32_t* tile_map, hipStream_t stream, int ks, float* ws, float* tail_ws,
+                            int handout) {
     const int ntm = fs2_cdiv(a.M, 256), ntn = fs2_cdiv(a.N, 128);
     const int cus = fs2_cu_count();
     PSched sc;
@@ -689,6 +761,9 @@
     const int taps = a.taps;
     sc.order = (ntn >= 2 && sc.G % 8 == 0 && (long)ntm * ntn * ks >= 2L * cus) ? 1 : 0;
     const bool wide = taps > 1 && (taps - 1) * a.dil > 16;
+    sc.la = p_lookahead(taps == 1 ? PCfg<true, false>::D : (wide ? PCfg<false, true>::D : PCfg<false, false>::D), taps, sc.nkc_u);
+    const bool dynamic = handout == FS2_HANDOUT_DYNAMIC || (handout == FS2_HANDOUT_AUTO && P_AUTO_DYNAMIC && (long)ntm * ntn * ks >= 2L * sc.G);
+    sc.cnt = dynamic ? p_slot_next(stream) : nullptr;
     if (a.in_act == FS2_ACT_LRELU) {
         if (taps == 1) launch_p<true, false, 1>(a, sc, stream);
         else if (wide) launch_p<false, true, 1>(a, sc, stream);
diff --git a/fastspeech2_amd/csrc/fs2_sched.h b/fastspeech2_amd/csrc/fs2_sched.h
--- a/fastspeech2_amd/csrc/fs2_sched.h
+++ b/fastspeech2_amd/csrc/fs2_sched.h
@@ -16,7 +16,10 @@
     float* tws;
     int tks_max;
     int order;
+    int32_t* cnt;
+    int la;
 };
+static constexpr int P_SLOT_WORDS = 16;
 
 struct PPlan { int Gg, j, x, T, R, tail, tks; };
 FS2_HD PPlan p_plan(const PSched& s, int b) {
@@ -65,6 +68,21 @@
     return true;
 }
 
+FS2_HD int p_static_pos(const PPlan& p, int k) { return (k < p.R ? k : p.R) * p.Gg + p.j; }
+FS2_HD bool p_unit_at(const PSched& s, const PPlan& p, int pos, bool tail_turn, int& mi, int& nt, int& kc0, int& nkc, int& np) {
+    if (pos < p.R * p.Gg) {
+        int sp;
+        p_pos(s, p, pos, mi, nt, sp);
+        np = 1; nkc = s.nkc_u; kc0 = sp * s.nkc_u;
+        return true;
+    }
+    return tail_turn && p_unit(s, p.R, mi, nt, kc0, nkc, np);
+}
+FS2_HD int p_lookahead(int D, int taps, int nkc_u) {
+    const int reach = D - 1 > taps ? D - 1 : taps;
+    return reach / (taps * nkc_u) + 1;
+}
+
 FS2_HD int p_max_units(int n_real, int ntn, int ks, int G, int order) {
     long T, Gg;
     if (order == 0) { T = (long)n_real * ntn * ks; Gg = G; }
diff --git a/fastspeech2_amd/ops.py b/fastspeech2_amd/ops.py
--- a/fastspeech2_amd/ops.py
+++ b/fastspeech2_amd/ops.py
@@ -158,6 +158,20 @@
     return y
 
 
+HANDOUT_AUTO, HANDOUT_STATIC, HANDOUT_DYNAMIC = -1, 0, 1
+
+
+def conv_gemm_p(x, wpacked, bias, S, taps=1, dil=1, pad=0, act=ACT_NONE, slope=0.0, lens=None, res=None, out=None, accumulate=False,
+                out_scale=1.0, tmap=None, ksplit=1, ws=None, tail_ws=None, handout=HANDOUT_AUTO):
+    M, Cin, N = x.shape[0], wpacked.shape[-1], wpacked.shape[0]
+    if out is None:
+        out = torch.empty(M, N, device=x.device, dtype=x.dtype)
+    _lib.call("fs2_conv_gemm_p", _p(x), x.stride(0), _p(wpacked), _p(bias), _p(res), res.stride(0) if res is not None else 0, _p(out),
+              out.stride(0), _p(lens), _p(tmap), _p(tail_ws), _p(ws), ksplit, handout, M, N, Cin, S, taps, dil, pad, act, slope,
+              int(accumulate), out_scale, dt(x), _stream())
+    return out
+
+
 def tail_workspace(device):
     return torch.empty(_lib.load().fs2_conv_gemm_tail_ws_bytes() // 4, device=device, dtype=torch.float32)
 
diff --git a/include/fs2hip.h b/include/fs2hip.h
--- a/include/fs2hip.h
+++ b/include/fs2hip.h
@@ -31,6 +31,14 @@
                          long ldy, const int32_t* lens, const int32_t* tile_map, float* ws, int ksplit, int M, int N, int Cin,
                          int S, int taps, int dil, int pad, int act, float slope, float out_scale, int dtype,
                          fs2_stream_t stream);
+#define FS2_HANDOUT_AUTO (-1)
+#define FS2_HANDOUT_STATIC 0
+#define FS2_HANDOUT_DYNAMIC 1
+int fs2_conv_gemm_p(const void* X, long ldx, const void* Wpacked, const float* bias, const void* R, long ldr, void* Y, long ldy,
+                    const int32_t* lens, const int32_t* tile_map, float* tail_ws, float* ws, int ksplit, int handout, int M, int N,
+                    int Cin, int S, int taps, int dil, int pad, int act, float slope, int accumulate, float out_scale, int dtype,
+                    fs2_stream_t stream);
+int fs2_conv_gemm_p_slots(void);
 int fs2_conv_gemm_lrelu_io(const void* X, long ldx, const void* Wpacked, const float* bias, const void* R, long ldr, void* Y,
                            long ldy, float* tail_ws, int M, int N, int Cin, int S, int taps, int dil, int pad, int act, float slope,
                            int accumulate, float out_scale, float res_unlrelu, float post_slope, int dtype, fs2_stream_t stream);
diff --git a/include/fs2hip_testaid.h b/include/fs2hip_testaid.h
--- a/include/fs2hip_testaid.h
+++ b/include/fs2hip_testaid.h
@@ -1,11 +1,18 @@
 #ifndef FS2HIP_TESTAID_H
 #define FS2HIP_TESTAID_H
+#include <stdint.h>
 #ifdef __cplusplus
 extern "C" {
 #endif
 int fs2t_stage_tile_col(int c, int elem_bytes);
 int fs2t_conv_gemm_p_units(int n_real, int ntn, int G, int order, int ks, int nkc, int tks_max, int b, int* out, int max_units);
 int fs2t_conv_gemm_p_max_units(int n_real, int ntn, int ks, int G, int order);
+int fs2t_conv_gemm_p_claim(int n_real, int ntn, int G, int order, int ks, int nkc, int tks_max, int b, int take, int32_t* slot,
+                           int* state, int* out);
+int fs2t_conv_gemm_p_exit(int G, int32_t* slot);
+int fs2t_conv_gemm_p_static_entry(int n_real, int ntn, int G, int order, int ks, int nkc, int tks_max, int b, int k, int* out);
+int fs2t_conv_gemm_p_lookahead(int D, int taps, int nkc_u);
+int fs2t_conv_gemm_p_slot_words(void);
 #ifdef __cplusplus
 }
 #endif
```

Measured after the change: 4.688 million mel-frames/s. No clear change (-0.1%).
